# facebookresearch/NeRF-Det

Hardware: AMD Instinct MI355X
Metric: scenes/sec (50-view 240x320, 40x40x16 voxels) (higher is better)
Workload: dtype f32 (convolutions: fp32 operands as hi + lo fp16 pairs of the power-of-two pre-scaled tensors, three products per multiply on the fp16 MFMA, fp32 accumulate; error against fp64 at or below the six-product bf16x3 form's; a device-side range guard repeats a scene on bf16x3 when part of a tensor falls ; 1 GPU; cfg2: nerfdet_res50_2x_low_res forward_test, 50 views 240x320, 40x40x16 voxels, fp32, 1 scene/step/GPU, random-init weights; parallelism=scene replicas x1 (no data-path collective)

## Files before the change

include/nerfdet_hip.h:

```cpp
#ifndef NERFDET_HIP_H
#define NERFDET_HIP_H

#include <stdint.h>

#ifdef __cplusplus
extern "C" {
#endif

#define NDET_OK 0
#define NDET_E_INVALID (-1)
#define NDET_E_UNSUPPORTED (-2)
#define NDET_E_LAUNCH (-3)

#define NDET_LAYOUT_CN 0
#define NDET_LAYOUT_NC 1

int ndet_version(void);
const char* ndet_last_error(void);

int ndet_get_points(float* points, int nx, int ny, int nz, const float* voxel_size_host,
                    const float* origin_host, void* stream);

int ndet_nchw_to_nhwc(const float* src, float* dst, int n, int c, int hw, void* stream);

int ndet_hbm_copy(const float* src, float* dst, int64_t n_floats, void* stream);

int ndet_backproject(const float* features, int n_views, int C, int h, int w,
                     int64_t sv, int64_t sc, int64_t sy, int64_t sx,
                     const float* points, int N, const float* projection,
                     float* volume, uint8_t* valid, void* stream);

int ndet_backproject_aggregate(const float* features_nhwc, int n_views, int C, int h, int w,
                               int64_t view_pitch, int64_t row_pitch,
                               const float* points, int N, const float* projection,
                               const float* alpha, float* out, int out_layout, int64_t* count,
                               void* stream);

int ndet_density_features(const float* mapped_nhwc, int n_views, int cm, int h, int w,
                          int64_t mview_pitch, int64_t mrow_pitch, const float* bias,
                          const float* rgb, int H, int W, int64_t rsv, int64_t rsc, int64_t rsy,
                          const float* points, int N, const float* projection, const float* rgb_projection,
                          float* global_feat, void* stream);

int ndet_density_features_packed(const float* mapped_nhwc, int n_views, int cm, int h, int w,
                                 int64_t mview_pitch, int64_t mrow_pitch, const float* bias,
                                 const float* rgb, int H, int W, int64_t rsv, int64_t rsc, int64_t rsy,
                                 const float* points, int N, const float* projection,
                                 const float* rgb_projection, float* global_feat, void* stream);

typedef struct NdetDepthGate {
    int32_t size;
    int32_t dtype;
    int32_t n_views;
    int32_t h, w;
    int32_t H, W;
    const void* depth_f;
    int64_t f_view_pitch, f_row_pitch;
    const void* depth_r;
    int64_t r_view_pitch, r_row_pitch;
    double band;
} NdetDepthGate;

int ndet_depth_resize(const void* depth, int dtype, int n_views, int Hd, int Wd, int64_t sv, int64_t sy,
                      void* out_f, int h, int w, void* out_r, int H, int W, void* stream);

int ndet_backproject_gated(const float* features, int n_views, int C, int h, int w,
                           int64_t sv, int64_t sc, int64_t sy, int64_t sx,
                           const float* points, int N, const float* projection,
                           float* volume, uint8_t* valid, const NdetDepthGate* gate, void* stream);

int ndet_backproject_aggregate_gated(const float* features_nhwc, int n_views, int C, int h, int w,
                                     int64_t view_pitch, int64_t row_pitch,
                                     const float* points, int N, const float* projection,
                                     const float* alpha, float* out, int out_layout, int64_t* count,
                                     const NdetDepthGate* gate, void* stream);

int ndet_density_features_gated(const float* mapped_nhwc, int n_views, int cm, int h, int w,
                                int64_t mview_pitch, int64_t mrow_pitch, const float* bias,
                                const float* rgb, int H, int W, int64_t rsv, int64_t rsc, int64_t rsy,
                                const float* points, int N, const float* projection, const float* rgb_projection,
                                float* global_feat, const NdetDepthGate* gate, void* stream);

int ndet_density_features_packed_gated(const float* mapped_nhwc, int n_views, int cm, int h, int w,
                                       int64_t mview_pitch, int64_t mrow_pitch, const float* bias,
                                       const float* rgb, int H, int W, int64_t rsv, int64_t rsc, int64_t rsy,
                                       const float* points, int N, const float* projection,
                                       const float* rgb_projection, float* global_feat, const NdetDepthGate* gate, void* stream);

typedef struct NdetSceneAccum {
    int32_t size;
    int32_t N, C, cm;
    int32_t n_views;
    float* k1_sum;
    int64_t k1_pitch;
    int32_t* k1_count;
    float* k2_sum;
    int64_t k2_pitch;
    int32_t* k2_count;
} NdetSceneAccum;

int ndet_scene_accumulate(const NdetSceneAccum* s, const float* features_nhwc, int n_views, int h, int w,
                          int64_t view_pitch, int64_t row_pitch, const float* mapped_nhwc, int64_t mview_pitch,
                          int64_t mrow_pitch, const float* bias, const float* rgb, int H, int W, int64_t rsv, int64_t rsc,
                          int64_t rsy, const float* points, const float* projection, const float* rgb_projection,
                          const NdetDepthGate* gate, void* stream);

int ndet_scene_density_finish(const NdetSceneAccum* s, const float* bias, float* global_feat, void* stream);

int ndet_scene_volume_finish(const NdetSceneAccum* s, const float* alpha, float* out, int64_t* count, void* stream);

#define NDET_RING_MAX 64

int ndet_scene_density_finish_ring(const NdetSceneAccum* segs, int n_segs, const float* bias, float* global_feat, void* stream);

int ndet_scene_volume_finish_ring(const NdetSceneAccum* segs, int n_segs, const float* alpha, float* out, int64_t* count, void* stream);

#define NDET_GROUP_MAX 64
typedef struct NdetSceneSlot {
    float* k1_sum;
    int32_t* k1_count;
    float* k2_sum;
    int32_t* k2_count;
    const float* points;
    int64_t reserved[3];
} NdetSceneSlot;

typedef struct NdetSceneGroup {
    int32_t size;
// ... 127 lines not shown

int ndet_sample_pdf(const float* bins, const float* weights, int R, int M, const float* u, int u_row_stride, int n_out, float* samples,
                    void* stream);

int ndet_importance_merge(const float* z_vals, const float* weights, const float* ray_o, const float* ray_d, int R, int S, const float* u,
                          int u_row_stride, int n_imp, float* z_out, float* pts_out, float* z_samples_out, void* stream);

int64_t ndet_conv3d_workspace_bytes(int D, int H, int W, int Cin, int Cout, int ksize, int stride, int splits);
int ndet_conv3d_ndhwc(const float* in, const float* w_packed, float* out, int D, int H, int W, int Cin, int Cout,
                      int ksize, int stride, int transposed, const float* scale, const float* shift,
                      const float* residual, int relu, int splits, int tile, void* workspace, void* stream);

int ndet_conv_ndhwc(const float* in, const float* w_packed, float* out, int D, int H, int W, int Cin, int Cout,
                    const int* kernel_host, const int* stride_host, const int* pad_host, const float* scale,
                    const float* shift, const float* residual, int residual_up2, int relu, int splits, int tile,
                    void* workspace, void* stream);

int ndet_split_weights_bf16x3(const float* w_packed, int taps, int Cout, int Cin, uint16_t* planes, void* stream);

int ndet_split_weights_bf16x3_torch(const float* w_torch, int taps, int Cout, int Cin, int adjoint, uint16_t* planes, void* stream);

int ndet_point_mlp_alpha(const float* points, const float* global_feat, int N, int F, int K0, int hidden, const uint16_t* const* w_planes_host,
                         const float* w_inv_scale_host, const float* const* bias_host, const float* w_sigma, const float* b_sigma,
                         float* raw_sigma, float* alpha, float* h_out, void* stream);

int ndet_split_weights_f16x2(const float* w_packed, int taps, int Cout, int Cin, float scale, uint16_t* planes, void* stream);

int ndet_amax_f32(const float* x, int64_t n, float* slot, void* stream);

int ndet_amax_slot_floats(void);

int ndet_measurement_knob(const char* name_host, int64_t value);

typedef struct NdetConvArgs {
    int32_t size;
    const float* in;
    const uint16_t* w_planes;
    float* out;
    int D, H, W, Cin, Cout;
    int kernel[3], stride[3], pad[3];
    int transposed;
    const float* scale;
    const float* shift;
    const float* residual;
    int residual_up2, relu, splits, tile, arith;
    const float* in_amax;
    float w_inv_scale;
    const float* w_amax;
    float* out_amax;
    void* workspace;
    unsigned* guard;
    float guard_l1, guard_tol;
    int keep_partials;
    const float* map_w;
    const float* map_b;
    float* map_out;
} NdetConvArgs;
int ndet_conv_split(const NdetConvArgs* a, void* stream);

int ndet_conv_split_batch(const NdetConvArgs* a, int batch, void* stream);

int ndet_conv_halo_patch(int tile, int D, int H, int W, const int* kernel, int* patch, int* looped);

#define NDET_TILE_DIRECT 1
#define NDET_TILE_OWNS_ROWS 2
#define NDET_TILE_ORDER2 4
int ndet_conv_tile_info(int tile, int* rows, int* cols, int* flags);

int ndet_conv_chain(const float* in, const uint16_t* w_planes, int D, int H, int W, int Cin, int Cmid, const int* kernel,
                    const int* stride, const int* pad, const float* scale1, const float* shift1, const uint16_t* w3_planes,
                    int Cout, const float* scale3, const float* shift3, const float* residual, int relu3, float* out,
                    int arith, const float* in_amax, float w1_inv_scale, float w3_inv_scale, float* out_amax, float guard_l1,
                    float guard_l1_3, float guard_tol, unsigned* guard, void* stream);

int ndet_bottleneck_f16x2(const float* x, int N, int H, int W, int Cin, int Cout, const uint16_t* w1_planes, float w1_inv_scale, const float* scale1,
                          const float* shift1, const uint16_t* w2_planes, float w2_inv_scale, const float* scale2, const float* shift2,
                          const uint16_t* w3_planes, float w3_inv_scale, const float* scale3, const float* shift3, const uint16_t* wd_planes,
                          float wd_inv_scale, const float* scale_d, const float* shift_d, const float* in_amax, float* out_amax, float* out,
                          const float* guard_l1_host, float guard_tol, unsigned* guard, void* stream);

int ndet_bn_relu_maxpool_nhwc(const float* x, const float* scale, const float* shift, int N, int H, int W, int C,
                              float* out, void* stream);

int ndet_stem_pack_weights(const float* w_64x3x7x7, uint16_t* planes , void* stream);
int ndet_stem_pack_weights_f16x2(const float* w_64x3x7x7, float scale, uint16_t* planes , void* stream);

int ndet_stem_conv_bn_relu_maxpool(const float* images, int N, int H, int W, int64_t stride_n, int64_t stride_c, int64_t stride_y,
                                   int64_t stride_x, const uint16_t* w_planes, float w_inv_scale, const float* scale, const float* shift, float* out, float* out_amax,
                                   void* stream);

int ndet_normalize_views(const uint8_t* frames_bgr, const int* ids, int n_sel, int H, int W, const double* mean_rgb,
                         const double* std_rgb, float* img, float* denorm, void* stream);

int ndet_target_rays(const uint8_t* frames_bgr, const int* target_ids, int n_targets, int H, int W, int margin,
                     const float* intrinsic_rows, const float* camrotc2w, const float* cam_lightpos, const double* mean_rgb,
                     const double* std_rgb, float* raydirs, float* lightpos, float* gt_images, void* stream);

int ndet_resize_normalize_views(const uint8_t* frames_bgr, const int* ids, int n_sel, int Hs, int Ws, int Hr, int Wr, int H, int W,
                                const double* mean_rgb, const double* std_rgb, float* img, float* denorm, uint8_t* resized_bgr,
                                void* stream);

int ndet_depth_frames(const uint16_t* frames_mm, const int* ids, int n_sel, int Hd, int Wd, int h, int w, int margin, double* out,
                      void* stream);

int ndet_positive_indices(const double* x, int64_t n, int64_t* indices, int64_t* count, void* workspace, void* stream);

// ... 83 lines not shown
```

nerf-det_amd/_lib.py:

```python
from __future__ import annotations

import ctypes
import os
from ctypes import c_char_p, c_float, c_int, c_int64, c_void_p

_HERE = os.path.dirname(os.path.abspath(__file__))
LIB_PATH = os.path.join(_HERE, "lib", "libnerfdet_hip.so")

NDET_LAYOUT_CN = 0
NDET_LAYOUT_NC = 1

_P = c_void_p
_F3 = ctypes.POINTER(c_float)


class NdetConvArgs(ctypes.Structure):
    _fields_ = ([("size", ctypes.c_int32), ("in_", _P), ("w_planes", _P), ("out", _P)] + [(f, c_int) for f in ("D", "H", "W", "Cin", "Cout")]
                + [(f, c_int * 3) for f in ("kernel", "stride", "pad")] + [("transposed", c_int), ("scale", _P), ("shift", _P), ("residual", _P)]
                + [(f, c_int) for f in ("residual_up2", "relu", "splits", "tile", "arith")] + [("in_amax", _P), ("w_inv_scale", c_float)]
                + [(f, _P) for f in ("w_amax", "out_amax", "workspace", "guard")] + [("guard_l1", c_float), ("guard_tol", c_float), ("keep_partials", c_int)]
                + [(f, _P) for f in ("map_w", "map_b", "map_out")])


class NdetDepthGate(ctypes.Structure):
    _fields_ = [(f, ctypes.c_int32) for f in ("size", "dtype", "n_views", "h", "w", "H", "W")] + [
        ("depth_f", _P), ("f_view_pitch", c_int64), ("f_row_pitch", c_int64),
        ("depth_r", _P), ("r_view_pitch", c_int64), ("r_row_pitch", c_int64), ("band", ctypes.c_double)]


class NdetSceneAccum(ctypes.Structure):
    _fields_ = [(f, ctypes.c_int32) for f in ("size", "N", "C", "cm", "n_views")] + [
        ("k1_sum", _P), ("k1_pitch", c_int64), ("k1_count", _P), ("k2_sum", _P), ("k2_pitch", c_int64), ("k2_count", _P)]


class NdetBankView(ctypes.Structure):
    _fields_ = [("feat", _P), ("rgb4", _P), ("ke", c_float * 12)]


NDET_GROUP_MAX = 64


class NdetSceneSlot(ctypes.Structure):
    _fields_ = [(f, _P) for f in ("k1_sum", "k1_count", "k2_sum", "k2_count", "points")] + [("reserved", c_int64 * 3)]


class NdetSceneGroup(ctypes.Structure):
    _fields_ = [(f, ctypes.c_int32) for f in ("size", "n_slots", "N", "C", "cm", "reserved")] + [
        ("k1_pitch", c_int64), ("k2_pitch", c_int64), ("table", _P)]


class NdetGroupSel(ctypes.Structure):
    _fields_ = [("size", ctypes.c_int32), ("n", ctypes.c_int32), ("slot", ctypes.c_int32 * NDET_GROUP_MAX),
                ("n_views", ctypes.c_int32 * NDET_GROUP_MAX)]


NDET_RING_MAX = 64
NDET_GROUP_POOL_MAX = NDET_GROUP_MAX * (NDET_RING_MAX + 1)


class NdetGroupRingSel(ctypes.Structure):
    _fields_ = [("size", ctypes.c_int32), ("n", ctypes.c_int32), ("n_segs", ctypes.c_int32 * NDET_GROUP_MAX),
                ("n_views", ctypes.c_int32 * NDET_GROUP_MAX)]


class NdetBankGroupSel(ctypes.Structure):
    _fields_ = [("size", ctypes.c_int32), ("n", ctypes.c_int32), ("views", _P * NDET_GROUP_MAX), ("n_views", ctypes.c_int32 * NDET_GROUP_MAX),
                ("n_points", ctypes.c_int32 * NDET_GROUP_MAX)]


_G = ctypes.POINTER(NdetDepthGate)
_GR = ctypes.POINTER(NdetGroupRingSel)
_S = ctypes.POINTER(NdetSceneAccum)
_SG = ctypes.POINTER(NdetSceneGroup)
_GS = ctypes.POINTER(NdetGroupSel)

SIGNATURES = {
    "ndet_version": ([], c_int),
    "ndet_last_error": ([], c_char_p),
    "ndet_get_points": ([_P, c_int, c_int, c_int, _F3, _F3, _P], c_int),
    "ndet_nchw_to_nhwc": ([_P, _P, c_int, c_int, c_int, _P], c_int),
    "ndet_hbm_copy": ([_P, _P, c_int64, _P], c_int),
    "ndet_backproject": ([_P, c_int, c_int, c_int, c_int, c_int64, c_int64, c_int64, c_int64, _P, c_int, _P, _P, _P, _P], c_int),
    "ndet_backproject_aggregate": ([_P, c_int, c_int, c_int, c_int, c_int64, c_int64, _P, c_int, _P, _P, _P, c_int, _P, _P], c_int),
    "ndet_density_features": ([_P, c_int, c_int, c_int, c_int, c_int64, c_int64, _P, _P, c_int, c_int, c_int64, c_int64,
                               c_int64, _P, c_int, _P, _P, _P, _P], c_int),
    "ndet_density_features_packed": ([_P, c_int, c_int, c_int, c_int, c_int64, c_int64, _P, _P, c_int, c_int, c_int64, c_int64,
                                      c_int64, _P, c_int, _P, _P, _P, _P], c_int),
    "ndet_depth_resize": ([_P, c_int, c_int, c_int, c_int, c_int64, c_int64, _P, c_int, c_int, _P, c_int, c_int, _P], c_int),
    "ndet_backproject_gated": ([_P, c_int, c_int, c_int, c_int, c_int64, c_int64, c_int64, c_int64, _P, c_int, _P, _P, _P, _G, _P], c_int),
    "ndet_backproject_aggregate_gated": ([_P, c_int, c_int, c_int, c_int, c_int64, c_int64, _P, c_int, _P, _P, _P, c_int, _P, _G, _P], c_int),
    "ndet_density_features_gated": ([_P, c_int, c_int, c_int, c_int, c_int64, c_int64, _P, _P, c_int, c_int, c_int64, c_int64,
                                     c_int64, _P, c_int, _P, _P, _P, _G, _P], c_int),
    "ndet_density_features_packed_gated": ([_P, c_int, c_int, c_int, c_int, c_int64, c_int64, _P, _P, c_int, c_int, c_int64, c_int64,
                                            c_int64, _P, c_int, _P, _P, _P, _G, _P], c_int),
    "ndet_backproject_aggregate_bwd_gated": ([_P, c_int, c_int, c_int, c_int, c_int, c_int64, c_int64, _P, c_int, _P, _P, _G, _P], c_int),
    "ndet_density_features_bwd_gated": ([_P, _P, c_int, c_int, c_int, c_int, c_int64, c_int64, _P, _P, c_int, _P, _P, _P, _G, _P], c_int),
    "ndet_scene_accumulate": ([_S, _P, c_int, c_int, c_int, c_int64, c_int64, _P, c_int64, c_int64, _P, _P, c_int, c_int, c_int64, c_int64, c_int64,
                               _P, _P, _P, _G, _P], c_int),
    "ndet_scene_density_finish": ([_S, _P, _P, _P], c_int),
    "ndet_scene_volume_finish": ([_S, _P, _P, _P, _P], c_int),
    "ndet_scene_density_finish_ring": ([_S, c_int, _P, _P, _P], c_int),
    "ndet_scene_volume_finish_ring": ([_S, c_int, _P, _P, _P, _P], c_int),
    "ndet_scene_group_check": ([_SG, _GS, c_int], c_int),
    "ndet_scene_accumulate_group": ([_SG, _GS, c_int, _P, c_int, c_int, c_int64, c_int64, _P, c_int64, c_int64, _P, _P, c_int, c_int, c_int64, c_int64,
                                     c_int64, _P, _P, _G, _P], c_int),
    "ndet_scene_density_finish_group": ([_SG, _GS, _P, _P, _P], c_int),
    "ndet_scene_volume_finish_group": ([_SG, _GS, _P, _P, _P, _P], c_int),
    "ndet_scene_group_ring_check": ([_SG, _GR, _P], c_int),
    "ndet_scene_density_finish_group_ring": ([_SG, _GR, _P, _P, _P, _P, _P], c_int),
    "ndet_scene_volume_finish_group_ring": ([_SG, _GR, _P, _P, _P, _P, _P, _P], c_int),
    "ndet_alpha_gate": ([_P, _P, _P, _P, c_int, c_int, c_int, _P], c_int),
    "ndet_sigma_to_alpha": ([_P, _P, c_int, _P], c_int),
    "ndet_posenc_concat": ([_P, _P, c_int, c_int, c_int, _P, _P], c_int),
    "ndet_sigma_head": ([_P, c_int, _P, c_int, c_int, _P, _P, c_int, _P, _P, _P], c_int),
    "ndet_nms_workspace_bytes": ([c_int], c_int64),
    "ndet_aligned_3d_nms": ([_P, _P, _P, c_int, c_float, _P, _P, _P, _P], c_int),
    "ndet_head_decode": ([_P, c_int, _P, _P, c_int, c_int, c_int, _F3, _F3, _P, _P, _P, _P], c_int),
    "ndet_head_decode_levels": ([c_int, _P, _P, _P, _P, _P, _P, c_int, _P, c_int, c_int, c_int, _P, _P, _P, _P], c_int),
    "ndet_sample_along_rays": ([_P, _P, c_int, c_int, c_float, c_float, _P, _P, _P, _P], c_int),
    "ndet_ray_view_stats": ([_P, c_int, _P, c_int, c_float, c_float, _P, c_int, c_int, c_int64, c_int64, c_int64,
                             _P, c_int, c_int, c_int, c_int64, c_int64, _P, _P, _P, _P], c_int),
    "ndet_pack_rgb_nhwc4": ([_P, c_int, c_int, c_int, c_int64, c_int64, c_int64, _P, _P], c_int),
    "ndet_ray_view_stats_packed": ([_P, c_int, _P, c_int, c_float, c_float, _P, c_int, c_int, _P, c_int, c_int, c_int, c_int64, c_int64,
                                    _P, _P, _P, _P], c_int),
    "ndet_ray_view_stats_bank": ([_P, c_int, _P, c_int, c_float, c_float, c_int, c_int, c_int, c_int, c_int, _P, _P, _P, _P], c_int),
    "ndet_ray_view_stats_bank_group": ([_P, ctypes.POINTER(NdetBankGroupSel), c_float, c_float, c_int, c_int, c_int, c_int, c_int, _P, _P, _P, _P], c_int),
    "ndet_ray_view_stats_packed_bwd": ([_P, _P, c_int, _P, c_int, c_float, c_float, _P, c_int, c_int, c_int, c_int64, c_int64, _P, _P], c_int),
    "ndet_project_sample": ([_P, c_int, _P, c_int, c_float, c_float, _P, c_int, c_int, c_int64, c_int64, c_int64,
                             _P, c_int, c_int, c_int, c_int64, c_int64, _P, _P, _P], c_int),
    "ndet_composite": ([_P, _P, _P, c_int, c_int, c_int, _P, _P, _P, _P, _P, _P, _P, _P], c_int),
    "ndet_sample_pdf": ([_P, _P, c_int, c_int, _P, c_int, c_int, _P, _P], c_int),
    "ndet_importance_merge": ([_P, _P, _P, _P, c_int, c_int, _P, c_int, c_int, _P, _P, _P, _P], c_int),
    "ndet_backproject_aggregate_bwd": ([_P, c_int, c_int, c_int, c_int, c_int, c_int64, c_int64, _P, c_int, _P, _P, _P], c_int),
    "ndet_density_features_bwd": ([_P, _P, c_int, c_int, c_int, c_int, c_int64, c_int64, _P, _P, c_int, _P, _P, _P, _P], c_int),
    "ndet_ray_view_stats_bwd": ([_P, _P, c_int, _P, c_int, c_float, c_float, _P, c_int, c_int, c_int, c_int64, c_int64, _P, _P], c_int),
    "ndet_composite_bwd": ([_P, _P, _P, c_int, c_int, c_int, _P, _P, _P, _P, _P], c_int),
    "ndet_split_weights_bf16x3": ([_P, c_int, c_int, c_int, _P, _P], c_int),
    "ndet_split_weights_f16x2": ([_P, c_int, c_int, c_int, c_float, _P, _P], c_int),
    "ndet_conv_split": ([ctypes.POINTER(NdetConvArgs), _P], c_int),
    "ndet_conv_split_batch": ([ctypes.POINTER(NdetConvArgs), c_int, _P], c_int),
    "ndet_conv_halo_patch": ([c_int] * 4 + [ctypes.POINTER(c_int)] * 3, c_int),
    "ndet_conv_tile_info": ([c_int] + [ctypes.POINTER(c_int)] * 3, c_int),
    "ndet_conv_chain": ([_P, _P] + [c_int] * 5 + [_P] * 6 + [c_int, _P, _P, _P, c_int, _P, c_int, _P, c_float, c_float, _P, c_float, c_float, c_float, _P, _P], c_int),
# ... 105 lines not shown
```

nerf-det_amd/conv3d.py:

```python
from __future__ import annotations

import ctypes
import math
import struct
from ctypes import c_void_p
from dataclasses import dataclass
from typing import Optional, Sequence

import torch
from torch import nn

from . import _lib, conv_tiles, trace
from ._lib import _ptr, check, i3, raw_stream
from .conv_tuning import TUNED, TUNED_BF16, TUNED_F16, TUNED_SPLIT

ARITHMETIC = "f16x2"
F16_MIN_KSTEPS = 4
SPLIT_FAMILY = ("bf16x3", "bf16", "f16x2")
ARITH_ID = {"bf16x3": 0, "f16x2": 1, "bf16": 2}


def set_arithmetic(mode: str) -> str:
    global ARITHMETIC
    if mode not in ("f32", "bf16x3", "bf16", "f16x2"):
# ... 123 lines not shown

def amax_value(slot: torch.Tensor) -> float:
    return float(slot.view(-1, 32)[:, 0].max())


def tilemin_value(slot: torch.Tensor) -> float:
    v = int(slot.view(torch.int32).view(-1, 32)[:, 1].max())
    return 0.0 if v == 0 else struct.unpack("<f", struct.pack("<I", 0x7f800000 - v))[0]


_slot_width_checked = False


def amax_of(x: torch.Tensor) -> torch.Tensor:
    global amax_fallbacks, _slot_width_checked
    if not _slot_width_checked:
        assert _lib.load().ndet_amax_slot_floats() == _AmaxSlots.WIDTH, "amax slot width of the library differs from conv3d._AmaxSlots.WIDTH"
        _slot_width_checked = True
    slot = _amax_tag(x)
    if slot is None:
        amax_fallbacks += 1
        slot = AMAX.take(x.device)
        st = c_void_p(raw_stream(x.device))
        check(_lib.load().ndet_amax_f32(_ptr(x), x.numel(), _ptr(slot), st), "amax_f32")
        _tag_amax(x, slot, produced=False)
    return slot


GUARD_ENABLED = True
GUARD_TOL = 2.0 ** -15
guard_trips = 0
_GUARD_WORDS = {}


def guard_word(device) -> Optional[torch.Tensor]:
    if not GUARD_ENABLED:
        return None
    key = (device, raw_stream(device))
    w = _GUARD_WORDS.get(key)
    if w is None:
        w = _GUARD_WORDS[key] = torch.zeros(1, dtype=torch.int32, device=device)
    return w


def guard_begin(device) -> None:
    w = guard_word(device)
    if w is not None:
        w.zero_()


def guard_tripped(device) -> bool:
    w = guard_word(device)
    return bool(w is not None and int(w.item()) & 1)


def guard_l1(pk: ConvPack) -> float:
    hit = pk.guard_l1
    if hit is None:
        w = pk.w.abs()
        wmax = w.max()
        tiny = ((w > 0) & (w < wmax * 2.0 ** -16)).sum(dim=(0, 2)).float()
        l1 = w.sum(dim=(0, 2)) + wmax * tiny
        if pk.scale is not None:
            l1 = l1 * pk.scale.abs()
        v = float(l1.max())
        hit = pk.guard_l1 = v if math.isfinite(v) else float("inf")
    return hit


launch_hook = None

KERNEL_NAMES = {("f32", 64): "k_conv3d_igemm<64,64,2,2>", ("f32", 128): "k_conv3d_igemm<128,128,4,2>"}
for _t, _row in conv_tiles.TILES.items():
    KERNEL_NAMES.update({("bf16x3", _t): _row.name, ("bf16", _t): _row.name, ("f16x2", _t): _row.name + "/f16x2"})


def _launch(flops, thunk, arith="f32", tile=0, nbytes=0, name=None):
    name = name or KERNEL_NAMES.get((arith, tile), f"{arith}:{tile}")
    if launch_hook is not None:
        return launch_hook(flops, thunk, name)
    return trace.span(name, thunk, flops=flops, bytes=nbytes, kind="conv")


def choose_tiling(m: int, cout: int, k_iters: int, tile: int = 0, splits: int = 0, transposed: bool = False):
    if tile == 0 and splits == 0:
        hit = TUNED.get((m, cout, k_iters, int(transposed)))
        if hit is not None:
            return hit
    if tile == 0:
        big = ((m + 127) // 128) * ((cout + 127) // 128)
        tile = 128 if (big >= 120 and cout >= 128 and k_iters > 4) else 64
    if splits == 0:
        if transposed:
            return tile, 1
        tiles = ((m + tile - 1) // tile) * ((cout + tile - 1) // tile)
        cap = 1200 if tile == 128 else 2400
        splits = 1
        while splits < 8 and k_iters // (splits + 1) >= 64 and tiles * (splits + 1) <= cap:
            splits += 1
    return tile, splits


def choose_tiling_split(m: int, cout: int, k_iters: int, tile: int = 0, splits: int = 0, transposed: bool = False, halo_ok: bool = False):
    if tile == 0 and splits in (0, 1):
        key = (m, cout, k_iters, int(transposed))
        hit = (TUNED_BF16.get(key) if ARITHMETIC == "bf16" else TUNED_F16.get(key) if ARITHMETIC == "f16x2" else None) or TUNED_SPLIT.get(key)
# ... 42 lines not shown


def f16_weight_scale(wmax: float) -> float:
    if not (wmax > 0.0 and math.isfinite(wmax)):
        return 1.0
    e = max(math.frexp(wmax)[1], -96)
    return math.ldexp(1.0, 15 - e)


def split_planes_f16(pk: ConvPack):
    hit = pk.planes_f16
    if hit is None:
        w = pk.w
        taps, cout, cin = w.shape
        if cin % 32:
            raise ValueError(f"conv_ndhwc_arith: Cin={cin} must be a multiple of 32")
        scale = f16_weight_scale(float(w.abs().max()))
        planes = torch.empty((taps, cin // 32, 2, cout, 32), dtype=torch.int16, device=w.device)
        st = c_void_p(raw_stream(w.device))
        check(_lib.load().ndet_split_weights_f16x2(_ptr(w), taps, cout, cin, scale, _ptr(planes), st), "split_weights_f16x2")
        hit = pk.planes_f16 = (planes, 1.0 / scale)
    return hit


def layer_arithmetic(k_iters: int) -> str:
    if ARITHMETIC == "f16x2" and k_iters < F16_MIN_KSTEPS:
        return "bf16x3"
    return ARITHMETIC


def _conv_split(x, pk, out, dims, kernel, stride, pad, transposed, residual, residual_up2, relu, splits, tile, m, k_iters, flops, want_amax=True, chain=None,
                keep_partials=False, batch=1):
    assert batch == 1 or (chain is None and not keep_partials and not residual_up2 and pk.w_amax is None)
    halo_ok = (not transposed and all(s == 1 for s in stride) and all(k % 2 == 1 and q == k // 2 for k, q in zip(kernel, pad))
               and kernel[0] * kernel[1] * kernel[2] > 1)
    tile, splits = choose_tiling_split(m, pk.cout, k_iters, tile, 1 if (transposed or residual_up2) else splits, transposed, halo_ok)
    tile, splits = conv_tiles.resolve(tile, splits, m=m, cout=pk.cout, cin=pk.cin, taps=kernel[0] * kernel[1] * kernel[2], transposed=transposed,
                                      halo_ok=halo_ok, direct_epilogue=DIRECT_EPILOGUE, batch=batch)
    ws = torch.empty((m * pk.cout * splits * 4,), dtype=torch.uint8, device=x.device) if splits > 1 else None
    st = c_void_p(raw_stream(x.device))
    lib = _lib.load()
    d, h, w = dims
    nbytes = 4 * (x.numel() + pk.w.numel() + out.numel() + (0 if residual is None else residual.numel()))
    arith = layer_arithmetic(k_iters)
    if ARITHMETIC == "f16x2" and pk.arith:
        arith = pk.arith
        want_amax = want_amax and pk.keep_amax
    if NO_AMAX_COMMIT:
        want_amax = False
    a = _lib.NdetConvArgs(size=ctypes.sizeof(_lib.NdetConvArgs), in_=x.data_ptr(), out=out.data_ptr(), D=d, H=h, W=w, Cin=pk.cin, Cout=pk.cout,
                          kernel=kernel, stride=stride, pad=pad, transposed=int(transposed), scale=_addr(pk.scale), shift=_addr(pk.shift),
                          residual=_addr(residual), residual_up2=int(residual_up2), relu=relu, splits=splits, tile=tile, arith=ARITH_ID[arith],
                          workspace=_addr(ws))
    keep, mapped = False, None
    if ARITHMETIC != "f16x2":
        a.w_planes = split_planes(pk).data_ptr()
        want_amax = False
    elif arith == "f16x2" and pk.w_amax is not None:
        assert not transposed and not residual_up2
        keep = keep_partials
        want_amax = want_amax and not keep
        a.w_planes, a.in_amax, a.w_amax, a.keep_partials = pk.planes_f16[0].data_ptr(), amax_of(x).data_ptr(), pk.w_amax.data_ptr(), int(keep)
        gw = guard_word(x.device) if pk.guard else None
        a.guard, a.guard_l1, a.guard_tol = _addr(gw), float(kernel[0] * kernel[1] * kernel[2] * pk.cin), GUARD_TOL
    else:
        if arith == "f16x2":
            planes, a.w_inv_scale = split_planes_f16(pk)
            a.in_amax = amax_of(x).data_ptr()
            gw = guard_word(x.device)
        else:
            planes, gw = split_planes(pk), None
        a.w_planes, a.guard, a.guard_l1, a.guard_tol = planes.data_ptr(), _addr(gw), (guard_l1(pk) if gw is not None else 0.0), GUARD_TOL
        if (chain is not None and conv_tiles.owns_rows(tile) and splits == 1 and residual is None and relu == 0 and not transposed and pk.cout == 256
                and arith in ("f16x2", "bf16x3")):
            mapped = torch.empty((m, 32), dtype=torch.float32, device=x.device)
            a.map_w, a.map_b, a.map_out = chain[0].data_ptr(), chain[1].data_ptr(), mapped.data_ptr()
            nbytes += 4 * mapped.numel()
    out_amax = AMAX.take(x.device) if want_amax else None
    a.out_amax = _addr(out_amax)
    if batch == 1:
        _launch(flops, lambda: check(lib.ndet_conv_split(a, st), "conv_split"), arith, tile, nbytes)
    else:
        _launch(flops, lambda: check(lib.ndet_conv_split_batch(a, batch, st), "conv_split_batch"), arith, tile, nbytes,
                name=KERNEL_NAMES.get((arith, tile), f"{arith}:{tile}") + "/batch")
    if want_amax:
        _tag_amax(out, out_amax)
    if keep_partials:
        return out, ((ws.view(torch.float32), splits) if keep and splits > 1 else None)
    return out if mapped is None else (out, mapped)


def projection_ok() -> bool:
    return ARITHMETIC == "f16x2"


def _addr(t):
    return None if t is None else t.data_ptr()


def pack_weight(w: torch.Tensor, transposed: bool = False) -> torch.Tensor:
    if w.dim() == 4:
        cout, cin = w.shape[:2]
        return w.permute(2, 3, 0, 1).reshape(-1, cout, cin).contiguous().float()
    if transposed:
        cin, cout = w.shape[:2]
        return w.permute(2, 3, 4, 1, 0).reshape(-1, cout, cin).contiguous().float()
# ... 317 lines not shown
```

nerf-det_amd/csrc/conv_common.hpp:

```cpp
#pragma once
#include <type_traits>
#include "ndet_common.hpp"

#define CBK 32

struct Conv3dParams {
    const float* in;
    const float* w;
    float* out;
    const float* scale;
    const float* shift;
    const float* res;
    float* partial;
    int D, H, W, Cin;
    int OD, OH, OW, Cout;
    int kd, kh, kw;
    int sd, sh, sw;
    int pd, ph, pw;
    int relu;
    int transposed;
    int splits;
    int M;
    int res_up2;
    int RH, RW;
    int max_order;
    int direct = 0;
    int order = 0;
    const float* amax_in = nullptr;
    float winv = 1.0f;
    const float* w_amax = nullptr;
    int nt = 0;
    float* amax_out = nullptr;
    const float* map_w = nullptr;
    const float* map_b = nullptr;
    float* map_out = nullptr;
    unsigned* guard = nullptr;
    float guard_l1 = 0.0f;
    float guard_tol = 0.0f;
};


#define NDET_AMAX_SUB 8
#define NDET_AMAX_STRIDE 32
__device__ __forceinline__ unsigned conv_xcc_id() { return __builtin_amdgcn_s_getreg((3 << 11) | 20) & 7u; }

__device__ __forceinline__ float conv_amax_read(const float* slot) {
    float v = slot[(threadIdx.x & (NDET_AMAX_SUB - 1)) * NDET_AMAX_STRIDE];
#pragma unroll
    for (int o = NDET_AMAX_SUB / 2; o; o >>= 1) v = fmaxf(v, __shfl_xor(v, o));
    return __uint_as_float(__builtin_amdgcn_readfirstlane(__float_as_uint(v)));
}

__device__ __forceinline__ float conv_xscale_of(float amax) {
    int eb = (int)((__float_as_uint(amax) >> 23) & 0xffu);
    eb = eb < 30 ? 30 : eb;
    return __uint_as_float((unsigned)(268 - eb) << 23);
}
__device__ __forceinline__ float conv_xinv_of(float amax) {
    int eb = (int)((__float_as_uint(amax) >> 23) & 0xffu);
    eb = eb < 30 ? 30 : eb;
    return __uint_as_float((unsigned)(eb - 14) << 23);
}
__device__ __forceinline__ float conv_xscale(const float* amax) { return conv_xscale_of(conv_amax_read(amax)); }
__device__ __forceinline__ float conv_winv(const Conv3dParams& p) { return p.w_amax ? conv_xinv_of(conv_amax_read(p.w_amax)) : p.winv; }
__device__ __forceinline__ float conv_oscale(const Conv3dParams& p) { return p.amax_in ? conv_xinv_of(conv_amax_read(p.amax_in)) * conv_winv(p) : 1.0f; }
__device__ __forceinline__ float conv_amax_in(const Conv3dParams& p) { return p.amax_in ? conv_amax_read(p.amax_in) : 0.0f; }
__device__ __forceinline__ float conv_oscale_of(const Conv3dParams& p, float amax_in) { return p.amax_in ? conv_xinv_of(amax_in) * conv_winv(p) : 1.0f; }

__device__ __forceinline__ void conv_amax_commit(float* slot, float mx) {
    __shared__ float wg_amax[16];
#pragma unroll
    for (int o = 32; o; o >>= 1) mx = fmaxf(mx, __shfl_xor(mx, o));
    const int nw = ((int)blockDim.x + 63) >> 6;
    if ((threadIdx.x & 63) == 0) wg_amax[threadIdx.x >> 6] = mx;
    __syncthreads();
    if (threadIdx.x == 0) {
        for (int i = 1; i < nw; ++i) mx = fmaxf(mx, wg_amax[i]);
        const unsigned bits = __float_as_uint(mx);
        unsigned* sub = reinterpret_cast<unsigned*>(slot) + conv_xcc_id() * NDET_AMAX_STRIDE;
        if (bits) atomicMax(sub, bits);
        if (bits && bits <= 0x7f800000u) atomicMax(sub + 1, 0x7f800000u - bits);
    }
}

__device__ __forceinline__ void conv_amax_commit_tiles(float* slot, float mx, float tmin) {
    __shared__ float wg_tmax[16], wg_tmin[16];
#pragma unroll
    for (int o = 32; o; o >>= 1) { mx = fmaxf(mx, __shfl_xor(mx, o)); tmin = fminf(tmin, __shfl_xor(tmin, o)); }
    const int nw = ((int)blockDim.x + 63) >> 6;
    if ((threadIdx.x & 63) == 0) { wg_tmax[threadIdx.x >> 6] = mx; wg_tmin[threadIdx.x >> 6] = tmin; }
    __syncthreads();
// ... 125 lines not shown
                                                int ztap, int zsplit, float& mx, float osc) {
    conv_store_rows_mapped<BN, NTHR>(p, Cs, cld, rows, n0, tid, ztap, zsplit, ConvLinearRows{m_first}, mx, osc);
}
template <int BN, int NTHR, typename RowMap>
__device__ __forceinline__ void conv_map_rows(const Conv3dParams& p, float* Cs, int cld, int tid, RowMap m_of, float osc, const float* Wl) {
    constexpr int KS = NTHR >= 1024 ? 8 : 4;
    static_assert(BN % KS == 0 && NTHR >= 128 * KS, "conv_map_rows: 128 threads per channel slice");
    constexpr int KQ = BN / KS;
    float acc[4][4];
#pragma unroll
    for (int i = 0; i < 4; ++i)
#pragma unroll
        for (int j = 0; j < 4; ++j) acc[i][j] = 0.f;
    const int kq = tid >> 7, rg = (tid >> 3) & 15, jg = tid & 7;
    if (tid < 128 * KS) {
        const float* c = Cs + rg * cld + kq * KQ;
        const float* w = Wl + (kq * KQ) * 32 + 4 * jg;
#pragma unroll 2
        for (int k = 0; k < KQ; ++k) {
            const float4 wv = *reinterpret_cast<const float4*>(w + k * 32);
#pragma unroll
            for (int i = 0; i < 4; ++i) {
                const float v = c[(16 * i) * cld + k];
                acc[i][0] = fmaf(v, wv.x, acc[i][0]); acc[i][1] = fmaf(v, wv.y, acc[i][1]);
                acc[i][2] = fmaf(v, wv.z, acc[i][2]); acc[i][3] = fmaf(v, wv.w, acc[i][3]);
            }
        }
    }
    __syncthreads();
    float* P = Cs;
    if (tid < 128 * KS) {
#pragma unroll
        for (int i = 0; i < 4; ++i)
            *reinterpret_cast<float4*>(P + ((kq * 64 + rg + 16 * i) * 32 + 4 * jg)) = make_float4(acc[i][0], acc[i][1], acc[i][2], acc[i][3]);
    }
    __syncthreads();
    for (int o = tid; o < 64 * 8; o += NTHR) {
        const int row = o >> 3, j4 = o & 7;
        const int m = m_of(row);
        if (m < 0 || m >= p.M) continue;
        float4 t = *reinterpret_cast<const float4*>(P + (row * 32 + 4 * j4));
#pragma unroll
        for (int q = 1; q < KS; ++q) {
            const float4 u = *reinterpret_cast<const float4*>(P + ((q * 64 + row) * 32 + 4 * j4));
            t.x += u.x; t.y += u.y; t.z += u.z; t.w += u.w;
        }
        const float4 b = *reinterpret_cast<const float4*>(p.map_b + 4 * j4);
        *reinterpret_cast<float4*>(p.map_out + (int64_t)m * 32 + 4 * j4) = make_float4(fmaf(t.x, osc, b.x), fmaf(t.y, osc, b.y), fmaf(t.z, osc, b.z), fmaf(t.w, osc, b.w));
    }
    __syncthreads();
}

__device__ __forceinline__ bool conv_writes_final(const Conv3dParams& p) { return p.transposed || p.splits <= 1; }
```

nerf-det_amd/csrc/conv_split_kernels.hip:

```cpp
#include "conv_common.hpp"

#include "spl_common.hpp"

#include <type_traits>

template <int BM, int BN, int WGM, int WGN, int SCH, bool BATCH = false>
__device__ __forceinline__ void conv_split_mainloop(const Conv3dParams& p, const uint16_t* __restrict__ wsplit, uint16_t* lds16,
                                                    f32x16 (&acc)[BM / WGM / 32][BN / WGN / 32], int& ztap) {
    constexpr int NTHR = 64 * WGM * WGN;
    constexpr int WM = BM / WGM, WN = BN / WGN;
    constexpr int MT = WM / 32, NT = WN / 32;
    constexpr int RPA = NTHR / 8;
    constexpr int RPB = NTHR / 4;
    constexpr int AR = BM / RPA, BR = BN / RPB;
    static_assert(AR >= 1 && BR >= 1 && MT >= 1 && NT >= 1, "tile too small for the thread count");
    constexpr int APL = BM * SPL_RS, BPL = BN * SPL_RS;
    constexpr int NPL = Spl<SCH>::NPL, WPL = Spl<SCH>::WPL;
    const float xs = SCH == 1 ? conv_xscale(p.amax_in) : 1.0f;
    uint16_t* As = lds16;
    uint16_t* Bs = lds16 + NPL * APL;

    const int tid = threadIdx.x;
    const int lane = tid & 63, wave = tid >> 6;
    const int wm = wave / WGN, wn = wave % WGN;
// ... 110 lines not shown
            uint16_t* dst = Bs + (brow_ + RPB * i) * SPL_RS + bkg * 8;
#pragma unroll
            for (int pl = 0; pl < NPL; ++pl) *reinterpret_cast<uint4*>(dst + pl * BPL) = rb[i][pl];
        }
    };

    if (it_begin < it_end) {
        load_tile();
        store_tile();
    }
    __syncthreads();

    const int frow = lane & 31, fk = (lane >> 5) * 8;
    const uint16_t* abase = As + (wm * WM + frow) * SPL_RS + fk;
    const uint16_t* bbase = Bs + (wn * WN + frow) * SPL_RS + fk;
    for (int it = it_begin; it < it_end; ++it) {
        const bool more = it + 1 < it_end;
        if (more) load_tile();
#pragma unroll
        for (int ks = 0; ks < CBK / 16; ++ks) {
            bf16x8 fa[NPL][MT], fb[NPL][NT];
#pragma unroll
            for (int pl = 0; pl < NPL; ++pl) {
                const int pq = NPL - 1 - pl;
#pragma unroll
                for (int t = 0; t < MT; ++t) fa[pl][t] = *reinterpret_cast<const bf16x8*>(abase + pl * APL + t * 32 * SPL_RS + ks * 16);
#pragma unroll
                for (int t = 0; t < NT; ++t) fb[pq][t] = *reinterpret_cast<const bf16x8*>(bbase + pq * BPL + t * 32 * SPL_RS + ks * 16);
            }
#pragma unroll
            for (int order = NPL - 1; order >= 0; --order)
                if (order <= p.max_order)
#pragma unroll
                for (int pa = 0; pa <= order; ++pa) {
                    const int pb = order - pa;
#pragma unroll
                    for (int ta = 0; ta < MT; ++ta)
#pragma unroll
                        for (int tb = 0; tb < NT; ++tb)
                            acc[ta][tb] = spl_mfma32<SCH>(fa[pa][ta], fb[pb][tb], acc[ta][tb]);
                }
        }
        __syncthreads();
        if (more) store_tile();
        __syncthreads();
    }
}

#ifndef UNI128_F16_WGS
#define UNI128_F16_WGS 3
#endif
template <int BM, int BN, int SCH> constexpr int uni_min_wgs() { return (SCH == 1 && BM == 128 && BN == 128) ? UNI128_F16_WGS : 2; }
#define SPL_BATCH 4
template <int BM, int BN, int WGM, int WGN, int SCHB = 0>
__global__ __launch_bounds__(64 * WGM * WGN, (uni_min_wgs<BM, BN, (SCHB & 3)>())) void k_conv_split(const Conv3dParams p, const uint16_t* __restrict__ wsplit) {
    constexpr int SCH = SCHB & 3;
    constexpr bool BATCH = (SCHB & SPL_BATCH) != 0;
    constexpr int NTHR = 64 * WGM * WGN;
    constexpr int WM = BM / WGM, WN = BN / WGN, MT = WM / 32, NT = WN / 32;
    extern __shared__ __attribute__((aligned(16))) uint16_t lds16[];
    const int tid = threadIdx.x;
    const int lane = tid & 63, wave = tid >> 6;
    const int wm = wave / WGN, wn = wave % WGN;
    const ConvBlock blk = conv_block(p);
    const int m0 = blk.x * BM, n0 = blk.y * BN;
    f32x16 acc[MT][NT];
    int ztap;
    const float amax_in = conv_amax_in(p);
    conv_guard_check(p, amax_in);
    conv_split_mainloop<BM, BN, WGM, WGN, SCH, BATCH>(p, wsplit, lds16, acc, ztap);
    const float osc = conv_oscale_of(p, amax_in);

    if (p.direct) {
        float mx = 0.0f;
        const unsigned obytes = (unsigned)((int64_t)p.M * p.Cout * 4);
        const unsigned rbytes = p.res_up2 ? (unsigned)((int64_t)p.OD * p.RH * p.RW * p.Cout * 4) : obytes;
        const __amdgpu_buffer_rsrc_t rres = __builtin_amdgcn_make_buffer_rsrc((void*)(p.res ? p.res : p.out), 0, p.res ? rbytes : obytes, 0x00020000);
        const __amdgpu_buffer_rsrc_t rout = __builtin_amdgcn_make_buffer_rsrc((void*)p.out, 0, obytes, 0x00020000);
#pragma unroll
        for (int tb = 0; tb < NT; ++tb) {
            const int co = n0 + wn * WN + tb * 32 + (lane & 31);
            if (n0 + wn * WN + tb * 32 >= p.Cout) continue;
            const float sc = p.scale ? p.scale[co] : 1.0f, sh = p.scale ? p.shift[co] : 0.0f;
#pragma unroll
            for (int ta = 0; ta < MT; ++ta) {
                const int mrow = m0 + wm * WM + ta * 32 + 4 * (lane >> 5);
                const unsigned vo = (unsigned)(((int64_t)mrow * p.Cout + co) * 4);
                float rr[16];
                if (p.res && p.res_up2) {
                    int uw = mrow % p.OW, uh = (mrow / p.OW) % p.OH, ud = mrow / (p.OW * p.OH);
#pragma unroll
                    for (int r = 0; r < 16; ++r) {
                        if (r) {
                            uw += (r & 3) ? 1 : 5;
                            if (p.OW >= 5) { if (uw >= p.OW) { uw -= p.OW; if (++uh == p.OH) { uh = 0; ++ud; } } }
                            else while (uw >= p.OW) { uw -= p.OW; if (++uh == p.OH) { uh = 0; ++ud; } }
                        }
                        const unsigned ro = ((((unsigned)ud * p.RH + (uh >> 1)) * p.RW + (uw >> 1)) * p.Cout + co) * 4u;
                        rr[r] = __uint_as_float(__builtin_amdgcn_raw_buffer_load_b32(rres, (mrow + (r & 3) + 8 * (r >> 2) < p.M) ? ro : 0xfffffff0u, 0, 0));
                    }
                } else {
#pragma unroll
                    for (int r = 0; r < 16; ++r) {
                        const unsigned so = __builtin_amdgcn_readfirstlane((unsigned)(((r & 3) + 8 * (r >> 2)) * p.Cout * 4));
                        rr[r] = p.res ? __uint_as_float(__builtin_amdgcn_raw_buffer_load_b32(rres, vo, so, 0)) : 0.0f;
                    }
                }
#pragma unroll
                for (int r = 0; r < 16; ++r) {
                    const unsigned so = __builtin_amdgcn_readfirstlane((unsigned)(((r & 3) + 8 * (r >> 2)) * p.Cout * 4));
                    float v = (acc[ta][tb][r] * osc) * sc + sh;
                    if (p.relu == 2) v = fmaxf(v, 0.f);
                    v += rr[r];
                    if (p.relu == 1) v = fmaxf(v, 0.f);
                    if (p.nt) __builtin_amdgcn_raw_buffer_store_b32(__float_as_uint(v), rout, vo, so, 2);
                    else __builtin_amdgcn_raw_buffer_store_b32(__float_as_uint(v), rout, vo, so, 0);
                    if (mrow + (r & 3) + 8 * (r >> 2) < p.M) mx = fmaxf(mx, fabsf(v));
                }
            }
        }
        if (p.amax_out) conv_amax_commit(p.amax_out, mx);
        return;
    }
    constexpr int CLDC = BN + 4;
    float* Cs = reinterpret_cast<float*>(lds16);
    float mx = 0.0f;
    for (int h = 0; h < WGM; ++h) {
        if (wm == h) {
#pragma unroll
            for (int ta = 0; ta < MT; ++ta)
#pragma unroll
                for (int tb = 0; tb < NT; ++tb)
#pragma unroll
                    for (int r = 0; r < 16; ++r)
                        Cs[(ta * 32 + (r & 3) + 8 * (r >> 2) + 4 * (lane >> 5)) * CLDC + wn * WN + tb * 32 + (lane & 31)] = acc[ta][tb][r];
        }
        __syncthreads();
        conv_store_rows<BN, NTHR>(p, Cs, CLDC, m0 + h * WM, WM, n0, tid, ztap, blk.z, mx, osc);
        __syncthreads();
    }
    if (p.amax_out && conv_writes_final(p)) conv_amax_commit(p.amax_out, mx);
}


struct ConvChain {
    const uint16_t* w3;
    float w3inv;
    float* amax_out;
    const float* scale3;
    const float* shift3;
    const float* res;
    float* out;
    int Cout3;
    int relu3;
    float guard_l1 = 0.0f;
};

#ifndef CHAIN64_F16_WGS
#define CHAIN64_F16_WGS 4
#endif
template <int MID, int SCH>
__global__ __launch_bounds__(256, MID == 64 ? (SCH == 1 ? CHAIN64_F16_WGS : 3) : 2) void k_conv_split_chain(const Conv3dParams p, const uint16_t* __restrict__ wsplit, const ConvChain c) {
    constexpr int BM = 128, BN = MID, WGM = 2, WGN = 2;
    constexpr int WM = BM / WGM, WN = BN / WGN, MT = WM / 32, NT = WN / 32;
    constexpr int NPL = Spl<SCH>::NPL, WPL = Spl<SCH>::WPL;
    constexpr int YRS = MID;
    constexpr int HALVES = MID == 128 ? 2 : 1;
    constexpr int RH = BM / HALVES;
    constexpr int YPL = RH * YRS;
    constexpr int NRT = RH / 32;
    constexpr int KS = MID / 16;
    constexpr int KG = 4, NKG = KS / KG;
    extern __shared__ __attribute__((aligned(16))) uint16_t lds16[];
    const int tid = threadIdx.x;
    const int lane = tid & 63, wave = __builtin_amdgcn_readfirstlane(tid >> 6);
    const int wm = wave / WGN, wn = wave % WGN;
    const int m0 = blockIdx.x * BM;
    f32x16 acc[MT][NT];
    int ztap;
    const float amax_in = conv_amax_in(p);
    conv_guard_check(p, amax_in);
    conv_split_mainloop<BM, BN, WGM, WGN, SCH>(p, wsplit, lds16, acc, ztap);
    const float osc = conv_oscale_of(p, amax_in);

    float ys = 1.0f, osc3 = 1.0f;
    if constexpr (SCH == 1) {
        const float osc1 = conv_oscale(p);
        float ymax = 0.0f;
#pragma unroll
        for (int ta = 0; ta < MT; ++ta)
#pragma unroll
            for (int tb = 0; tb < NT; ++tb) {
// ... 290 lines not shown
                    fa[pl][t] = *reinterpret_cast<const bf16x8*>(abase + pl * APL + t * 32 * SPL_RS + (((2 * ks + (lane >> 5)) ^ (((wm * WM + t * 32 + frow) >> 4) & 3)) << 3));
#pragma unroll
                for (int t = 0; t < NT; ++t) fb[pl][t] = *reinterpret_cast<const bf16x8*>(bbase + pl * BPL + t * 32 * SPL_RS + ks * 16);
            }
#pragma unroll
            for (int order = NPL - 1; order >= 0; --order)
                if (order <= p.max_order)
#pragma unroll
                for (int pa = 0; pa <= order; ++pa) {
                    const int pb = order - pa;
#pragma unroll
                    for (int ta_ = 0; ta_ < MT; ++ta_)
#pragma unroll
                        for (int tb_ = 0; tb_ < NT; ++tb_)
                            acc[ta_][tb_] = spl_mfma32<SCH>(fa[pa][ta_], fb[pb][tb_], acc[ta_][tb_]);
                }
        }
        __syncthreads();
        if (more) store_tile();
        __syncthreads();
    }
    constexpr int CLDC = BN + 4;
    float* Cs = reinterpret_cast<float*>(lds16);
    for (int h = 0; h < WGM; ++h) {
        if (wm == h) {
#pragma unroll
            for (int ta_ = 0; ta_ < MT; ++ta_)
#pragma unroll
                for (int tb_ = 0; tb_ < NT; ++tb_)
#pragma unroll
                    for (int r = 0; r < 16; ++r)
                        Cs[(ta_ * 32 + (r & 3) + 8 * (r >> 2) + 4 * (lane >> 5)) * CLDC + wn * WN + tb_ * 32 + (lane & 31)] = acc[ta_][tb_][r];
        }
        __syncthreads();
        float mx_unused = 0.0f;
        conv_store_rows<BN, NTHR>(p, Cs, CLDC, m0 + h * WM, WM, n0, tid, 0, bz, mx_unused, osc);
        __syncthreads();
    }
}


typedef unsigned int u32x4 __attribute__((ext_vector_type(4)));
typedef float f32x4v __attribute__((ext_vector_type(4)));
__device__ __forceinline__ int ws_swz(int row) { return (row >> 1) & 2; }
__device__ __forceinline__ void spl_dma16(__amdgpu_buffer_rsrc_t rsrc, uint16_t* lds_dst, unsigned voffset, unsigned soffset) {
    __builtin_amdgcn_raw_ptr_buffer_load_lds(rsrc, (__attribute__((address_space(3))) void*)lds_dst, 16, voffset, soffset, 0, 0);
}

#define WS_BM 128
#define WS_BN 256
#define WS_DEPTH 2
#define WS_OOB 0x80000000u

template <int SCHB>
__global__ __launch_bounds__(512, 1) void k_conv_split_ws(const Conv3dParams p, const uint16_t* __restrict__ wsplit) {
    constexpr int SCH = SCHB & 3;
    constexpr bool BATCH = (SCHB & SPL_BATCH) != 0;
    constexpr int APL = WS_BM * CBK, BPL = WS_BN * CBK;
    constexpr int NPL = Spl<SCH>::NPL, WPL = Spl<SCH>::WPL;
    constexpr int STAGE = NPL * (APL + BPL);
    constexpr int AR = 4, BR = 4;
    extern __shared__ __attribute__((aligned(16))) uint16_t lds16[];

    const int tid = threadIdx.x;
    const int lane = tid & 63;
    const int wave = __builtin_amdgcn_readfirstlane(tid >> 6);
    const bool consumer = wave < 4;
    const int wm = (wave & 3) >> 1, wn = wave & 1;
    const ConvBlock blk = conv_block(p);
    const int m0 = blk.x * WS_BM, n0 = blk.y * WS_BN;
    const float amax_in = conv_amax_in(p);
    conv_guard_check(p, amax_in);
    const int stid = tid & 255;
    const int akq = stid & 7, arow_ = stid >> 3;
    const int bkg = stid & 3, brow_ = stid >> 2;

    const int cin_steps = p.Cin / CBK;
    const int wkd = p.transposed ? 1 : p.kd, wkh = p.transposed ? 1 : p.kh, wkw = p.transposed ? 1 : p.kw;
    const int taps = wkd * wkh * wkw;
    const int n_iters_all = taps * cin_steps;
    int it_begin = 0, it_end = n_iters_all;
    int ztap = 0;
    if (p.transposed) {
        ztap = blk.z;
    } else if (p.splits > 1) {
        const int s = blk.z;
        it_begin = (int)((int64_t)n_iters_all * s / p.splits);
        it_end = (int)((int64_t)n_iters_all * (s + 1) / p.splits);
    }
    const int n_it = it_end - it_begin;
    const int n_round = (n_it + WS_DEPTH - 1) / WS_DEPTH * WS_DEPTH;

    f32x4v acc[4][8];
#pragma unroll
    for (int a = 0; a < 4; ++a)
#pragma unroll
        for (int b = 0; b < 8; ++b) acc[a][b] = (f32x4v){0.f, 0.f, 0.f, 0.f};

    if (!consumer) {
        const int64_t shift = p.transposed ? 0 : (((int64_t)p.pd * p.H + p.ph) * p.W + p.pw) * p.Cin;
        const __amdgpu_buffer_rsrc_t ares = __builtin_amdgcn_make_buffer_rsrc((void*)(p.in - shift), 0, WS_OOB, 0x00020000);
        const __amdgpu_buffer_rsrc_t bres = __builtin_amdgcn_make_buffer_rsrc((void*)wsplit, 0, WS_OOB, 0x00020000);
        unsigned avoff[AR], amask[AR];
#pragma unroll
        for (int i = 0; i < AR; ++i) {
            const int m = m0 + arow_ + 32 * i;
            const bool vok = m < p.M;
// ... 117 lines not shown
        }
    } else {
        const int frow = lane & 15, fc = lane >> 4;
        const int kc = (fc ^ ws_swz(frow)) * 8;
        const int aoff = (wm * 64 + frow) * CBK + kc;
        const int boff = NPL * APL + (wn * 128 + frow) * CBK + kc;
        __syncthreads();
        for (int j = 0; j < n_round; ++j) {
            if (j < n_it) {
                const uint16_t* st = lds16 + (j & 1) * STAGE;
                bf16x8 fa[NPL][4], fb[NPL][8];
#pragma unroll
                for (int pl = 0; pl < NPL; ++pl) {
                    const int pq = NPL - 1 - pl;
#pragma unroll
                    for (int t = 0; t < 4; ++t) fa[pl][t] = *reinterpret_cast<const bf16x8*>(st + aoff + pl * APL + t * 16 * CBK);
#pragma unroll
                    for (int t = 0; t < 8; ++t) fb[pq][t] = *reinterpret_cast<const bf16x8*>(st + boff + pq * BPL + t * 16 * CBK);
                }
#pragma unroll
                for (int order = NPL - 1; order >= 0; --order)
                    if (order <= p.max_order)
#pragma unroll
                    for (int pa = 0; pa <= order; ++pa) {
                        const int pb = order - pa;
#pragma unroll
                        for (int ta = 0; ta < 4; ++ta)
#pragma unroll
                            for (int tb = 0; tb < 8; ++tb)
                                acc[ta][tb] = spl_mfma16<SCH>(fa[pa][ta], fb[pb][tb], acc[ta][tb]);
                    }
            }
            __syncthreads();
        }
    }

    constexpr int CLDC = WS_BN + 4;
    float* Cs = reinterpret_cast<float*>(lds16);
    float mx = 0.0f;
    for (int h = 0; h < 2; ++h) {
        if (consumer && wm == h) {
#pragma unroll
            for (int ta = 0; ta < 4; ++ta)
#pragma unroll
                for (int tb = 0; tb < 8; ++tb)
#pragma unroll
                    for (int r = 0; r < 4; ++r)
                        Cs[(ta * 16 + (lane >> 4) * 4 + r) * CLDC + wn * 128 + tb * 16 + (lane & 15)] = acc[ta][tb][r];
        }
        __syncthreads();
        conv_store_rows<WS_BN, 512>(p, Cs, CLDC, m0 + h * 64, 64, n0, tid, ztap, blk.z, mx, conv_oscale_of(p, amax_in));
        __syncthreads();
    }
    if (p.amax_out && conv_writes_final(p)) conv_amax_commit(p.amax_out, mx);
}

static inline int conv_scheme(const Conv3dParams& p) { return p.max_order == 0 ? 2 : (p.max_order == 1 ? 1 : 0); }

template <class F>
static inline int with_scheme(int sch, F&& f) {
    return sch == 2 ? f(std::integral_constant<int, 2>{}) : (sch == 1 ? f(std::integral_constant<int, 1>{}) : f(std::integral_constant<int, 0>{}));
}

template <bool BATCH>
static int split_launch_ws_n(const Conv3dParams& p, int batch, hipStream_t st, const char* fn) {
    const int taps = p.transposed ? 1 : p.kd * p.kh * p.kw;
    const int64_t nvol = BATCH ? batch : 1;
    NDET_REQUIRE(taps <= 32, NDET_E_UNSUPPORTED, "%s: the 128x256 tile supports at most 32 taps", fn);
    NDET_REQUIRE(nvol * p.D * p.H * p.W * p.Cin * 4 < ((int64_t)1 << 31) && (int64_t)(p.transposed ? 8 : taps) * p.Cin * p.Cout * 6 < ((int64_t)1 << 31),
                 NDET_E_UNSUPPORTED, "%s: the 128x256 tile addresses at most 2 GB per operand", fn);
    const int zdim = p.transposed ? 8 : p.splits;
    dim3 grid((p.M + WS_BM - 1) / WS_BM, (p.Cout + WS_BN - 1) / WS_BN, zdim);
    const int sch = conv_scheme(p);
    size_t lds = (size_t)2 * (sch == 2 ? 1 : (sch == 1 ? 2 : 3)) * (WS_BM + WS_BN) * CBK * sizeof(uint16_t);
    const size_t cs = (size_t)64 * (WS_BN + 4) * sizeof(float);
    if (cs > lds) lds = cs;
    return with_scheme(sch, [&](auto s) -> int {
        const auto kernel = k_conv_split_ws<decltype(s)::value + (BATCH ? SPL_BATCH : 0)>;
        NDET_RAISE_LDS(kernel, lds);
        hipLaunchKernelGGL(kernel, grid, dim3(512), lds, st, p, (const uint16_t*)p.w);
        return NDET_OK;
    });
}
static int split_launch_ws(const Conv3dParams& p, hipStream_t st, const char* fn) { return split_launch_ws_n<false>(p, 1, st, fn); }
static int split_launch_ws_batch(const Conv3dParams& p, int batch, hipStream_t st, const char* fn) { return split_launch_ws_n<true>(p, batch, st, fn); }


template <int OFF>
__device__ __forceinline__ void lds_store64_unseen(unsigned addr, uint2 v) {
    const unsigned long long d = ((unsigned long long)v.y << 32) | v.x;
    asm volatile("ds_write_b64 %0, %1 offset:%2" ::"v"(addr), "v"(d), "n"(OFF) : "memory");
}

#ifndef WSP_DEPTH
#define WSP_DEPTH 2
#endif
template <int SCH, int BM, int NCONS>
__global__ __launch_bounds__(64 * (NCONS + 4), 1) void k_conv_split_wsp(const Conv3dParams p, const uint16_t* __restrict__ wsplit, int n_mt, int n_nt) {
    static_assert((BM == 128 && (NCONS == 4 || NCONS == 8)) || (BM == 64 && NCONS == 4), "consumer layouts: 2 x 2 of 64 x 128, 2 x 4 of 64 x 64, 1 x 4 of 64 x 64");
    constexpr int CW = NCONS / (BM / 64);
    constexpr int WNC = WS_BN / CW, NTB = WNC / 16;
    constexpr int APL = BM * CBK, BPL = WS_BN * CBK;
    constexpr int NPL = Spl<SCH>::NPL, WPL = Spl<SCH>::WPL;
    constexpr int STAGE = NPL * (APL + BPL);
    extern __shared__ __attribute__((aligned(16))) uint16_t lds16[];

    const int tid = threadIdx.x;
    const int lane = tid & 63;
    const int wave = __builtin_amdgcn_readfirstlane(tid >> 6);
    const bool consumer = wave < NCONS;
    const float xs = SCH == 1 ? conv_xscale(p.amax_in) : 1.0f;
    const float osc = conv_oscale(p);
    if (SCH == 1) conv_guard_check(p, conv_amax_in(p));
    __shared__ float s_tmax[2][NCONS];
    const bool track = p.amax_out != nullptr && p.splits == 1;
    float mx = 0.0f, tmin = INFINITY;
    int kt = 0;
    auto fold_tile = [&](int k) {
        float m = s_tmax[k & 1][0];
#pragma unroll
        for (int i = 1; i < NCONS; ++i) m = fmaxf(m, s_tmax[k & 1][i]);
        if (m > 0.0f) tmin = fminf(tmin, m);
    };
    const int wm = (wave % NCONS) / CW, wn = (wave % NCONS) % CW;

    const int cin_steps = p.Cin / CBK;
    const int wkd = p.kd, wkh = p.kh, wkw = p.kw;
    const int taps = wkd * wkh * wkw;
    const int n_iters_all = taps * cin_steps;
    const int n_tiles = n_mt * n_nt * p.splits;
    const int G = gridDim.x;
// ... 241 lines not shown
    NDET_REQUIRE(taps <= 32, NDET_E_UNSUPPORTED, "%s: the persistent 128x256 tile supports at most 32 taps", fn);
    NDET_REQUIRE(p.Cout % 16 == 0, NDET_E_UNSUPPORTED, "%s: the persistent 128x256 tile needs Cout %% 16 == 0", fn);
    NDET_REQUIRE((int64_t)p.D * p.H * p.W * p.Cin * 4 < ((int64_t)1 << 31) && (int64_t)taps * p.Cin * p.Cout * 6 < ((int64_t)1 << 31) &&
                     ((int64_t)p.M + 128) * p.Cout * 4 < ((int64_t)1 << 31),
                 NDET_E_UNSUPPORTED, "%s: the persistent 128x256 tile addresses at most 2 GB per operand", fn);
    const int n_mt = (p.M + BM - 1) / BM, n_nt = (p.Cout + WS_BN - 1) / WS_BN;
    const int64_t n_tiles = (int64_t)n_mt * n_nt * p.splits;
    static int n_cu = 0;
    if (n_cu == 0) {
        int dev = 0;
        hipDeviceProp_t prop;
        if (hipGetDevice(&dev) != hipSuccess || hipGetDeviceProperties(&prop, dev) != hipSuccess) n_cu = 256;
        else n_cu = prop.multiProcessorCount > 0 ? prop.multiProcessorCount : 256;
    }
    const int grid = (int)(n_tiles < n_cu ? n_tiles : n_cu);
    const int sch = conv_scheme(p);
    const size_t lds = (size_t)2 * (sch == 2 ? 1 : (sch == 1 ? 2 : 3)) * (BM + WS_BN) * CBK * sizeof(uint16_t);
    return with_scheme(sch, [&](auto s) -> int {
        const auto kernel = k_conv_split_wsp<decltype(s)::value, BM, NCONS>;
        NDET_RAISE_LDS(kernel, lds);
        hipLaunchKernelGGL(kernel, dim3(grid), dim3(64 * (NCONS + 4)), lds, st, p, (const uint16_t*)p.w, n_mt, n_nt);
        return NDET_OK;
    });
}


struct HaloGeom {
    int ltd, lth, ltw;
    int npd, nph, npw;
    int HH, HW, NH;
    int T;
    int KDL;
    int Tin;
};

struct HaloRowMap {
    int first, ltw, lth, d0, h0, w0, OD, OH, OW;
    __device__ __forceinline__ int operator()(int row) const {
        const int r = first + row;
        const int tw = r & ((1 << ltw) - 1), th = (r >> ltw) & ((1 << lth) - 1), td = r >> (ltw + lth);
        const int od = d0 + td, oh = h0 + th, ow = w0 + tw;
        return (od < OD && oh < OH && ow < OW) ? (od * OH + oh) * OW + ow : -1;
    }
};
struct HaloRowMapBatch {
    HaloRowMap in_volume;
    int vol_first;
    __device__ __forceinline__ int operator()(int row) const {
        const int m = in_volume(row);
        return m < 0 ? m : vol_first + m;
    }
};

template <int NT16, int WGN, int SCHB, int NPROD = 4>
__global__ __launch_bounds__(64 * (2 * WGN + NPROD), 1) void k_conv_split_halo(const Conv3dParams p, const uint16_t* __restrict__ wsplit, const HaloGeom g) {
    constexpr int SCH = SCHB & 3;
    constexpr bool BATCH = (SCHB & SPL_BATCH) != 0;
    constexpr int BN = 16 * NT16 * WGN;
    constexpr int NCONS = 2 * WGN, NTHR = 64 * (NCONS + NPROD);
    constexpr int PT = 64 * NPROD;
    constexpr int HALO_MAX = (BN == 128) ? 400 : 224;
    constexpr int NSTAGE = (BN == 128) ? 3 : 2;
    constexpr int NPIECE = (HALO_MAX * 8 + PT - 1) / PT;
    constexpr int APL = HALO_MAX * CBK, BPL = BN * CBK;
    constexpr int NPL = SCH == 1 ? 2 : (SCH == 2 ? 1 : 3);
    constexpr int WPL = SCH == 1 ? 2 : 3;
    constexpr int BSTAGE = NPL * BPL;
    constexpr int BR = BN / (16 * NPROD);
    static_assert(BR >= 1 && BN % (16 * NPROD) == 0, "every producer wave stages 16 rows of each row group");
    constexpr int NB = NPL * BR;
    extern __shared__ __attribute__((aligned(16))) uint16_t lds16[];
    uint16_t* Bs = lds16 + NPL * APL;

    const int tid = threadIdx.x;
    const int lane = tid & 63;
    const int wave = __builtin_amdgcn_readfirstlane(tid >> 6);
    const bool consumer = wave < NCONS;
    const int wm = (wave % NCONS) / WGN, wn = (wave % NCONS) % WGN;
    const ConvBlock blk = conv_block(p);
    const int n0 = blk.y * BN;
    const int TH = 1 << g.lth, TW = 1 << g.ltw;
    int pb = blk.x;
    const int pwi = pb % g.npw; pb /= g.npw;
    const int phi = pb % g.nph;
    const int pdv = pb / g.nph;
    const int vol = BATCH ? pdv / g.npd : 0;
    const int pdi = BATCH ? pdv - vol * g.npd : pdv;
    const int d0 = pdi << g.ltd, h0 = phi << g.lth, w0 = pwi << g.ltw;
    const float amax_in = conv_amax_in(p);
    conv_guard_check(p, amax_in);

    const int nch_all = p.Cin / CBK;
    int cb = 0, ce = nch_all;
    if (p.splits > 1) {
        cb = (int)((int64_t)nch_all * blk.z / p.splits);
        ce = (int)((int64_t)nch_all * (blk.z + 1) / p.splits);
    }
    const int nch = ce - cb;
    const int T = g.T, Tin = g.Tin;
    const int S = nch * T;
    const int nphase = nch * g.KDL;

    f32x4v acc[4][NT16];
#pragma unroll
    for (int a = 0; a < 4; ++a)
#pragma unroll
        for (int b = 0; b < NT16; ++b) acc[a][b] = (f32x4v){0.f, 0.f, 0.f, 0.f};
// ... 127 lines not shown
                    const int pq = NPL - 1 - pl;
#pragma unroll
                    for (int ta = 0; ta < 4; ++ta) fa[pl][ta] = *reinterpret_cast<const bf16x8*>(ap[ta] + pl * APL);
#pragma unroll
                    for (int tb = 0; tb < NT16; ++tb) fb[pq][tb] = *reinterpret_cast<const bf16x8*>(bst + pq * BPL + tb * 16 * CBK);
                }
#pragma unroll
                for (int order = NPL - 1; order >= 0; --order)
                    if (order <= p.max_order)
#pragma unroll
                    for (int pa = 0; pa <= order; ++pa) {
                        const int pbb = order - pa;
#pragma unroll
                        for (int ta = 0; ta < 4; ++ta)
#pragma unroll
                            for (int tb = 0; tb < NT16; ++tb) {
                                acc[ta][tb] = spl_mfma16<SCH>(fa[pa][ta], fb[pbb][tb], acc[ta][tb]);
                            }
                    }
                if (++kw == wkw) {
                    kw = 0;
                    if (++kh == wkh) { kh = 0; ++kd; }
                }
                __syncthreads();
            }
            if (ci + 1 < nphase) __syncthreads();
        }
    }
    __builtin_amdgcn_s_setprio(0);

    constexpr int CLDC = BN + 4;
    float* Cs = reinterpret_cast<float*>(lds16);
    float mx = 0.0f;
    for (int h = 0; h < 2; ++h) {
        if (consumer && wm == h) {
#pragma unroll
            for (int ta = 0; ta < 4; ++ta)
#pragma unroll
                for (int tb = 0; tb < NT16; ++tb)
#pragma unroll
                    for (int r = 0; r < 4; ++r)
                        Cs[(ta * 16 + (lane >> 4) * 4 + r) * CLDC + wn * (16 * NT16) + tb * 16 + (lane & 15)] = acc[ta][tb][r];
        }
        __syncthreads();
        const HaloRowMap rmap{h * 64, g.ltw, g.lth, d0, h0, w0, p.OD, p.OH, p.OW};
        const float osc = conv_oscale_of(p, amax_in);
        float* Wl = Cs + 64 * CLDC;
        if (p.map_out && h == 0)
            for (int i = tid; i < BN * 8; i += NTHR) reinterpret_cast<float4*>(Wl)[i] = reinterpret_cast<const float4*>(p.map_w)[i];
        if constexpr (BATCH) conv_store_rows_mapped<BN, NTHR>(p, Cs, CLDC, 64, n0, tid, 0, blk.z, HaloRowMapBatch{rmap, vol * p.OD * p.OH * p.OW}, mx, osc);
        else conv_store_rows_mapped<BN, NTHR>(p, Cs, CLDC, 64, n0, tid, 0, blk.z, rmap, mx, osc);
        __syncthreads();
        if (p.map_out) conv_map_rows<BN, NTHR>(p, Cs, CLDC, tid, rmap, osc, Wl);
    }
    if (p.amax_out && conv_writes_final(p)) conv_amax_commit(p.amax_out, mx);
}

static bool halo_geometry(const Conv3dParams& p, int halo_max, HaloGeom& g) {
    double best = 1e30;
    for (int dloop = 0; dloop <= (p.kd > 1 ? 1 : 0); ++dloop)
        for (int ltd = 0; ltd <= 7; ++ltd)
            for (int lth = 0; lth + ltd <= 7; ++lth) {
                const int ltw = 7 - ltd - lth;
                const int TD = 1 << ltd, TH = 1 << lth, TW = 1 << ltw;
                const int HD = dloop ? TD : TD + p.kd - 1, HH = TH + p.kh - 1, HW = TW + p.kw - 1;
                const int NH = HD * HH * HW;
                if (NH > halo_max) continue;
                const int npd = (p.OD + TD - 1) / TD, nph = (p.OH + TH - 1) / TH, npw = (p.OW + TW - 1) / TW;
                const double waste = (double)npd * TD * nph * TH * npw * TW / ((double)p.OD * p.OH * p.OW);
                const int kdl = dloop ? p.kd : 1;
                const double cost = waste * (1.0 + 0.03 * NH * kdl / 128.0);
                if (cost < best) {
                    best = cost;
                    g.ltd = ltd; g.lth = lth; g.ltw = ltw; g.npd = npd; g.nph = nph; g.npw = npw; g.HH = HH; g.HW = HW; g.NH = NH;
                    g.KDL = kdl;
                }
            }
    g.T = p.kd * p.kh * p.kw;
    g.Tin = g.T / (best < 1e29 ? g.KDL : 1);
    return best < 1e29;
}

template <int NT16, int WGN, int SCH, int NPROD, bool BATCH>
static int split_launch_halo(const Conv3dParams& p, int batch, hipStream_t st, const char* fn) {
    constexpr int NPL = SCH == 1 ? 2 : (SCH == 2 ? 1 : 3);
    constexpr int BN = 16 * NT16 * WGN, HALO_MAX = (BN == 128) ? 400 : 224, NSTAGE = (BN == 128) ? 3 : 2;
    NDET_REQUIRE(!p.transposed && p.sd == 1 && p.sh == 1 && p.sw == 1 && (p.kd & 1) && (p.kh & 1) && (p.kw & 1) && p.pd == p.kd / 2 &&
                     p.ph == p.kh / 2 && p.pw == p.kw / 2,
                 NDET_E_UNSUPPORTED, "%s: the halo tile needs a stride-1 same-padded convolution with odd kernel extents", fn);
    const int64_t nvol = BATCH ? batch : 1;
    NDET_REQUIRE(nvol * p.D * p.H * p.W * p.Cin * 4 < ((int64_t)1 << 31) && (int64_t)p.kd * p.kh * p.kw * p.Cin * p.Cout * 6 < ((int64_t)1 << 31),
                 NDET_E_UNSUPPORTED, "%s: the halo tile addresses at most 2 GB per operand", fn);
    NDET_REQUIRE(p.splits <= p.Cin / CBK, NDET_E_INVALID, "%s: the halo tile splits K over the %d channel chunks only", fn, p.Cin / CBK);
    HaloGeom g;
    NDET_REQUIRE(halo_geometry(p, HALO_MAX, g), NDET_E_UNSUPPORTED, "%s: no patch shape fits the halo tile", fn);
    dim3 grid((unsigned)(nvol * g.npd * g.nph * g.npw), (p.Cout + BN - 1) / BN, p.splits);
    size_t lds = (size_t)(NPL * HALO_MAX * CBK + NSTAGE * NPL * BN * CBK) * sizeof(uint16_t);
    const size_t cs = (size_t)64 * (BN + 4) * sizeof(float);
    if (cs > lds) lds = cs;
    const size_t lds_map = cs + (size_t)BN * 32 * sizeof(float);
    const size_t lds_cap = lds_map > lds ? lds_map : lds;
    if (p.map_out) {
        NDET_REQUIRE(p.Cout == BN && p.splits == 1 && !p.res && p.relu == 0, NDET_E_UNSUPPORTED,
                     "%s: the chained projection needs a tile that owns all %d output channels of its rows, no split-K / residual / ReLU", fn, p.Cout);
        lds = lds_cap;
    }
    const auto kernel = k_conv_split_halo<NT16, WGN, SCH + (BATCH ? SPL_BATCH : 0), NPROD>;
    NDET_RAISE_LDS(kernel, lds_cap);
    hipLaunchKernelGGL(kernel, grid, dim3(64 * (2 * WGN + NPROD)), lds, st, p, (const uint16_t*)p.w, g);
    return NDET_OK;
}

template <int BM, int BN, int WGM, int WGN, int SCH, bool BATCH>
static int split_launch_tile_sch(const Conv3dParams& p, hipStream_t st, const char* fn) {
    const int zdim = p.transposed ? 8 : p.splits;
    dim3 grid((p.M + BM - 1) / BM, (p.Cout + BN - 1) / BN, zdim);
    size_t lds = (size_t)Spl<SCH>::NPL * (BM + BN) * SPL_RS * sizeof(uint16_t);
    const size_t cs = (size_t)(BM / WGM) * (BN + 4) * sizeof(float);
    if (cs > lds) lds = cs;
    const auto kernel = k_conv_split<BM, BN, WGM, WGN, SCH + (BATCH ? SPL_BATCH : 0)>;
    if (lds > 64 * 1024) NDET_RAISE_LDS(kernel, lds);
    hipLaunchKernelGGL(kernel, grid, dim3(64 * WGM * WGN), lds, st, p, (const uint16_t*)p.w);
    return NDET_OK;
}
template <int BM, int BN, int WGM, int WGN>
static int split_launch_tile(const Conv3dParams& p, hipStream_t st, const char* fn) {
    return with_scheme(conv_scheme(p), [&](auto s) { return split_launch_tile_sch<BM, BN, WGM, WGN, decltype(s)::value, false>(p, st, fn); });
}
template <int BM, int BN, int WGM, int WGN>
static int split_launch_tile_batch(const Conv3dParams& p, int, hipStream_t st, const char* fn) {
    return with_scheme(conv_scheme(p), [&](auto s) { return split_launch_tile_sch<BM, BN, WGM, WGN, decltype(s)::value, true>(p, st, fn); });
}
template <int NT16, int WGN>
static int split_launch_halo_any(const Conv3dParams& p, hipStream_t st, const char* fn) {
    return with_scheme(conv_scheme(p), [&](auto s) { return split_launch_halo<NT16, WGN, decltype(s)::value, 4, false>(p, 1, st, fn); });
}
template <int NT16, int WGN>
static int split_launch_halo_any_batch(const Conv3dParams& p, int batch, hipStream_t st, const char* fn) {
    return with_scheme(conv_scheme(p), [&](auto s) { return split_launch_halo<NT16, WGN, decltype(s)::value, 4, true>(p, batch, st, fn); });
}
static int split_launch_halo_p8(const Conv3dParams& p, hipStream_t st, const char* fn) {
    return with_scheme(conv_scheme(p), [&](auto s) {
        constexpr int SCH = decltype(s)::value;
        return split_launch_halo<4, 4, SCH, SCH == 0 ? 4 : 8, false>(p, 1, st, fn);
    });
}
static int split_launch_halo_p8_batch(const Conv3dParams& p, int batch, hipStream_t st, const char* fn) {
    return with_scheme(conv_scheme(p), [&](auto s) {
        constexpr int SCH = decltype(s)::value;
        return split_launch_halo<4, 4, SCH, SCH == 0 ? 4 : 8, true>(p, batch, st, fn);
    });
}

#ifndef NDET_ORDER_DEFAULT
#define NDET_ORDER_DEFAULT -1
#endif
static int64_t g_nt_bytes = (int64_t)32 << 20;
static bool g_order2 = true;
static int64_t conv_nt_bytes() { return g_nt_bytes; }
static int g_wgrad_wide = 1;
static int g_wgrad_xcd = 1;

extern "C" int ndet_measurement_knob(const char* name, int64_t value) {
    const char* fn = "ndet_measurement_knob";
    NDET_REQUIRE(name, NDET_E_INVALID, "%s: null name", fn);
    if (!strcmp(name, "nt_bytes")) { NDET_REQUIRE(value >= 0, NDET_E_INVALID, "%s: nt_bytes must be >= 0", fn); g_nt_bytes = value; return NDET_OK; }
    if (!strcmp(name, "order2")) { NDET_REQUIRE(value == 0 || value == 1, NDET_E_INVALID, "%s: order2 is 0 or 1", fn); g_order2 = value != 0; return NDET_OK; }
    if (!strcmp(name, "deterministic_scatter")) { NDET_REQUIRE(value == 0 || value == 1, NDET_E_INVALID, "%s: deterministic_scatter is 0 or 1", fn); g_ndet_deterministic_scatter = (int)value; return NDET_OK; }
    if (!strcmp(name, "wgrad_wide")) { NDET_REQUIRE(value == 0 || value == 1, NDET_E_INVALID, "%s: wgrad_wide is 0 or 1", fn); g_wgrad_wide = (int)value; return NDET_OK; }
    if (!strcmp(name, "wgrad_xcd")) { NDET_REQUIRE(value == 0 || value == 1, NDET_E_INVALID, "%s: wgrad_xcd is 0 or 1", fn); g_wgrad_xcd = (int)value; return NDET_OK; }
    ndet_set_error("%s: unknown knob '%s' (nt_bytes, order2, deterministic_scatter, wgrad_wide, wgrad_xcd)", fn, name);
    return NDET_E_INVALID;
}
extern "C" int ndet_amax_slot_floats(void) { return NDET_AMAX_SUB * NDET_AMAX_STRIDE; }

struct ConvTile {
    int id, rows, cols, flags;
    int (*launch)(const Conv3dParams&, hipStream_t, const char*);
    int (*launch_batch)(const Conv3dParams&, int batch, hipStream_t, const char*);
};
static const ConvTile CONV_TILES[] = {
    {64, 64, 64, NDET_TILE_ORDER2, split_launch_tile<64, 64, 2, 2>, split_launch_tile_batch<64, 64, 2, 2>},
    {128, 128, 128, NDET_TILE_ORDER2, split_launch_tile<128, 128, 2, 2>, split_launch_tile_batch<128, 128, 2, 2>},
    {12864, 128, 64, NDET_TILE_ORDER2, split_launch_tile<128, 64, 2, 2>, split_launch_tile_batch<128, 64, 2, 2>},
    {100064, 64, 64, NDET_TILE_ORDER2 | NDET_TILE_DIRECT, split_launch_tile<64, 64, 2, 2>, split_launch_tile_batch<64, 64, 2, 2>},
    {100128, 128, 128, NDET_TILE_ORDER2 | NDET_TILE_DIRECT, split_launch_tile<128, 128, 2, 2>, split_launch_tile_batch<128, 128, 2, 2>},
    {112864, 128, 64, NDET_TILE_ORDER2 | NDET_TILE_DIRECT, split_launch_tile<128, 64, 2, 2>, split_launch_tile_batch<128, 64, 2, 2>},
    {128256, 128, 256, NDET_TILE_ORDER2, split_launch_ws, split_launch_ws_batch},
    {129256, 128, 256, 0, split_launch_wsp<128, 4>, nullptr},
    {129257, 128, 256, 0, split_launch_wsp<128, 8>, nullptr},
    {129064, 64, 256, 0, split_launch_wsp<64, 4>, nullptr},
    {3128, 128, 128, 0, split_launch_halo_any<4, 2>, split_launch_halo_any_batch<4, 2>},
    {3256, 128, 256, NDET_TILE_OWNS_ROWS, split_launch_halo_any<8, 2>, split_launch_halo_any_batch<8, 2>},
    {3257, 128, 256, NDET_TILE_OWNS_ROWS, split_launch_halo_any<4, 4>, split_launch_halo_any_batch<4, 4>},
    {3258, 128, 256, NDET_TILE_OWNS_ROWS, split_launch_halo_p8, split_launch_halo_p8_batch},
};
static const ConvTile* conv_tile(int id) {
    for (const ConvTile& t : CONV_TILES)
        if (t.id == id) return &t;
    return nullptr;
}

extern "C" int ndet_conv_tile_info(int tile, int* rows, int* cols, int* flags) {
    const char* fn = "ndet_conv_tile_info";
    NDET_REQUIRE(rows && cols && flags, NDET_E_INVALID, "%s: null pointer", fn);
    const ConvTile* t = conv_tile(tile);
    NDET_REQUIRE(t, NDET_E_INVALID, "%s: unknown tile %d", fn, tile);
    *rows = t->rows; *cols = t->cols; *flags = t->flags;
    return NDET_OK;
}

extern "C" int ndet_conv_halo_patch(int tile, int D, int H, int W, const int* kernel, int* patch, int* looped) {
    const char* fn = "ndet_conv_halo_patch";
    NDET_REQUIRE(kernel && patch && looped, NDET_E_INVALID, "%s: null pointer", fn);
    const ConvTile* t = conv_tile(tile);
    NDET_REQUIRE(t && (tile == 3128 || (t->flags & NDET_TILE_OWNS_ROWS)), NDET_E_INVALID, "%s: tile %d is not a halo tile", fn, tile);
    NDET_REQUIRE(D > 0 && H > 0 && W > 0 && kernel[0] >= 1 && kernel[1] >= 1 && kernel[2] >= 1, NDET_E_INVALID, "%s: sizes must be positive", fn);
    Conv3dParams p{};
    p.OD = D; p.OH = H; p.OW = W; p.kd = kernel[0]; p.kh = kernel[1]; p.kw = kernel[2];
    HaloGeom g;
    NDET_REQUIRE(halo_geometry(p, t->cols == 128 ? 400 : 224, g), NDET_E_UNSUPPORTED, "%s: no patch shape fits the halo tile", fn);
    patch[0] = 1 << g.ltd; patch[1] = 1 << g.lth; patch[2] = 1 << g.ltw;
    *looped = g.KDL > 1 ? 1 : 0;
    return NDET_OK;
}

static int conv_split_launch_n(Conv3dParams& p, int tile, bool keep_partials, int batch, hipStream_t st, const char* fn) {
    p.nt = (p.splits <= 1 || p.transposed) && (int64_t)p.M * p.Cout * 4 * (p.transposed ? 8 : 1) >= conv_nt_bytes() ? 1 : 0;
    const int64_t big_tiles = (int64_t)((p.M + 127) / 128) * ((p.Cout + 127) / 128);
    if (tile == 0) tile = (big_tiles >= 192 && p.Cout >= 128) ? 128 : 64;
    const ConvTile* t = conv_tile(tile);
    NDET_REQUIRE(t, NDET_E_INVALID, "%s: unknown tile %d", fn, tile);
    NDET_REQUIRE(batch == 1 || t->launch_batch, NDET_E_UNSUPPORTED, "%s: tile %d takes one volume per launch", fn, tile);
    p.direct = (t->flags & NDET_TILE_DIRECT) ? 1 : 0;
    NDET_REQUIRE(!p.direct || (!p.transposed && p.splits == 1 && p.Cout % 32 == 0 && ((int64_t)p.M + 128) * p.Cout * 4 < ((int64_t)1 << 32)),
                 NDET_E_UNSUPPORTED, "%s: the direct epilogue needs splits == 1, no transposition, Cout %% 32 == 0 and an output below 4 GB", fn);
    {
        const int tm = t->rows, tn = t->cols;
        const int64_t mt = (p.M + tm - 1) / tm, nt = (p.Cout + tn - 1) / tn;
        const int64_t taps = p.transposed ? 1 : (int64_t)p.kd * p.kh * p.kw;
        const int64_t w_bytes = taps * p.Cin * p.Cout * 6, a_bytes = (int64_t)p.M * p.Cin * 4 * (p.sd * p.sh * p.sw);
        const int64_t save_w = (mt - 1) * w_bytes, save_a = (nt - 1) * a_bytes;
        p.order = NDET_ORDER_DEFAULT;
        if (NDET_ORDER_DEFAULT < 0) {
            p.order = 0;
            if (!p.transposed && mt > 1 && nt * p.splits > 1 && save_w > save_a && w_bytes > (8 << 20)) p.order = 1;
            if (g_order2 && p.order == 0 && !p.transposed && nt > 1 && mt >= 16 && w_bytes <= (2 << 20) && save_a >= (8 << 20) &&
                (t->flags & NDET_TILE_ORDER2)) p.order = 2;
        }
    }
    const int rc = batch == 1 ? t->launch(p, st, fn) : t->launch_batch(p, batch, st, fn);
    if (rc != NDET_OK) return rc;
    NDET_CHECK_LAUNCH(fn);
    if (keep_partials && p.splits > 1) return NDET_OK;
    return conv_splitk_reduce_launch(p, st, fn);
}
int conv_split_launch(Conv3dParams& p, int tile, bool keep_partials, hipStream_t st, const char* fn) {
    return conv_split_launch_n(p, tile, keep_partials, 1, st, fn);
}

__global__ __launch_bounds__(256) void k_split_weights(const float* __restrict__ w, int taps, int Cout, int Cin, uint16_t* __restrict__ out) {
    const int64_t i = ((int64_t)blockIdx.x * blockDim.x + threadIdx.x) * 2;
    const int64_t n = (int64_t)taps * Cout * Cin;
    if (i >= n) return;
    const int ci = (int)(i % Cin), co = (int)((i / Cin) % Cout), tap = (int)(i / ((int64_t)Cin * Cout));
    const float a = w[i], b = w[i + 1];
    const uint32_t o0 = spl_pack(a, b);
    const float ra = a - spl_lo(o0), rb = b - spl_hi(o0);
    const uint32_t o1 = spl_pack(ra, rb);
    const uint32_t o2 = spl_pack(ra - spl_lo(o1), rb - spl_hi(o1));
    const uint32_t o[3] = {o0, o1, o2};
    const int steps = Cin / CBK;
    uint16_t* dst = out + (((int64_t)tap * steps + ci / CBK) * 3 * Cout + co) * CBK + (ci % CBK);
#pragma unroll
    for (int pl = 0; pl < 3; ++pl) *reinterpret_cast<uint32_t*>(dst + (int64_t)pl * Cout * CBK) = o[pl];
}

extern "C" int ndet_split_weights_bf16x3(const float* w_packed, int taps, int Cout, int Cin, uint16_t* planes, void* stream) {
    const char* fn = "ndet_split_weights_bf16x3";
    NDET_REQUIRE(w_packed && planes, NDET_E_INVALID, "%s: null pointer", fn);
    NDET_REQUIRE(taps > 0 && Cout > 0 && Cin > 0, NDET_E_INVALID, "%s: sizes must be positive", fn);
    NDET_REQUIRE(Cin % CBK == 0, NDET_E_UNSUPPORTED, "%s: Cin=%d must be a multiple of %d", fn, Cin, CBK);
    const int64_t work = (int64_t)taps * Cout * Cin / 2;
    hipLaunchKernelGGL(k_split_weights, dim3((unsigned)((work + 255) / 256)), dim3(256), 0, (hipStream_t)stream, w_packed, taps, Cout, Cin, planes);
    NDET_CHECK_LAUNCH(fn);
    return NDET_OK;
}

__global__ __launch_bounds__(256) void k_split_weights_f16x2(const float* __restrict__ w, int taps, int Cout, int Cin, float scale, uint16_t* __restrict__ out) {
    const int64_t i = ((int64_t)blockIdx.x * blockDim.x + threadIdx.x) * 2;
    const int64_t n = (int64_t)taps * Cout * Cin;
    if (i >= n) return;
    const int ci = (int)(i % Cin), co = (int)((i / Cin) % Cout), tap = (int)(i / ((int64_t)Cin * Cout));
    const float a = w[i] * scale, b = w[i + 1] * scale;
    const uint32_t o0 = spl_pack_f16(a, b);
    const uint32_t o1 = spl_pack_f16(a - spl_f16_lo(o0), b - spl_f16_hi(o0));
    const int steps = Cin / CBK;
    uint16_t* dst = out + (((int64_t)tap * steps + ci / CBK) * 2 * Cout + co) * CBK + (ci % CBK);
    *reinterpret_cast<uint32_t*>(dst) = o0;
    *reinterpret_cast<uint32_t*>(dst + (int64_t)Cout * CBK) = o1;
}

extern "C" int ndet_split_weights_f16x2(const float* w_packed, int taps, int Cout, int Cin, float scale, uint16_t* planes, void* stream) {
    const char* fn = "ndet_split_weights_f16x2";
    NDET_REQUIRE(w_packed && planes, NDET_E_INVALID, "%s: null pointer", fn);
    NDET_REQUIRE(taps > 0 && Cout > 0 && Cin > 0 && scale > 0.0f, NDET_E_INVALID, "%s: sizes and scale must be positive", fn);
    NDET_REQUIRE(Cin % CBK == 0, NDET_E_UNSUPPORTED, "%s: Cin=%d must be a multiple of %d", fn, Cin, CBK);
// ... 178 lines not shown
    p.M = p.OD * p.OH * p.OW;
    return NDET_OK;
}

static int max_order_of(int arith) { return arith == 0 ? 2 : (arith == 1 ? 1 : 0); }

static int conv_split_entry(const NdetConvArgs* a, int batch, void* stream, const char* fn) {
    NDET_REQUIRE(a && a->size == (int32_t)sizeof(NdetConvArgs), NDET_E_INVALID, "%s: the argument block must be set up with size = %d", fn,
                 (int)sizeof(NdetConvArgs));
    NDET_REQUIRE(a->arith >= 0 && a->arith <= 2, NDET_E_INVALID, "%s: arith must be 0 (bf16x3), 1 (fp16 pair) or 2 (bf16)", fn);
    const bool f16 = a->arith == 1, train = a->w_amax != nullptr;
    NDET_REQUIRE(!train || (f16 && !a->transposed && !a->residual_up2), NDET_E_INVALID,
                 "%s: w_amax (the training form) needs arith 1, no transposition and no upsampled residual", fn);
    if (f16) {
        NDET_REQUIRE(a->in_amax && (train || a->w_inv_scale > 0.0f), NDET_E_INVALID,
                     "%s: the fp16-pair arithmetic needs the input's amax slot and the weight planes' inverse scale (or w_amax)", fn);
        NDET_REQUIRE(!a->guard || (a->guard_l1 >= 0.0f && a->guard_tol > 0.0f), NDET_E_INVALID, "%s: the guard needs guard_l1 >= 0 and guard_tol > 0", fn);
    } else {
        NDET_REQUIRE(!a->in_amax, NDET_E_INVALID, "%s: in_amax belongs to the fp16-pair arithmetic only", fn);
    }
    NDET_REQUIRE(!a->keep_partials || (!a->scale && !a->residual && !a->relu && !a->out_amax && !a->transposed), NDET_E_INVALID,
                 "%s: keep_partials leaves the epilogue to ndet_wgrad_to_torch (no affine / residual / ReLU / amax, no transposition)", fn);
    if (a->map_w || a->map_b || a->map_out) {
        NDET_REQUIRE(a->map_w && a->map_b && a->map_out, NDET_E_INVALID, "%s: null projection pointers", fn);
        NDET_REQUIRE((((uintptr_t)a->map_w | (uintptr_t)a->map_b | (uintptr_t)a->map_out) & 15) == 0, NDET_E_UNSUPPORTED,
                     "%s: projection pointers must be 16-byte aligned", fn);
        const ConvTile* t = conv_tile(a->tile);
        NDET_REQUIRE(t && (t->flags & NDET_TILE_OWNS_ROWS), NDET_E_UNSUPPORTED, "%s: tile %d does not own whole rows (3256 / 3257 / 3258 do)", fn, a->tile);
        NDET_REQUIRE(a->Cout == 256, NDET_E_UNSUPPORTED, "%s: Cout=%d, the 256-column tiles own whole rows of 256 channels only", fn, a->Cout);
        NDET_REQUIRE(a->splits <= 1 && !a->residual && !a->relu && !a->transposed, NDET_E_UNSUPPORTED,
                     "%s: the chained projection takes no split-K, residual, ReLU or transposition", fn);
    }
    if (batch != 1) {
        NDET_REQUIRE(batch >= 1, NDET_E_INVALID, "%s: batch=%d must be at least 1", fn, batch);
        NDET_REQUIRE(!a->w_amax && !a->keep_partials && !a->residual_up2 && !a->map_w && !a->map_b && !a->map_out, NDET_E_UNSUPPORTED,
                     "%s: a batch takes no w_amax, keep_partials, upsampled residual or chained projection", fn);
        const ConvTile* t = conv_tile(a->tile);
        NDET_REQUIRE(!t || t->launch_batch, NDET_E_UNSUPPORTED, "%s: tile %d (persistent) takes one volume per launch", fn, a->tile);
    }
    NDET_REQUIRE(a->in && a->w_planes && a->out, NDET_E_INVALID, "%s: null pointer", fn);
    NDET_REQUIRE(a->D > 0 && a->H > 0 && a->W > 0 && a->Cin > 0 && a->Cout > 0, NDET_E_INVALID, "%s: sizes must be positive", fn);
    NDET_REQUIRE((a->scale == nullptr) == (a->shift == nullptr), NDET_E_INVALID, "%s: scale and shift go together", fn);
    NDET_REQUIRE(a->relu >= 0 && a->relu <= 2, NDET_E_INVALID, "%s: bad relu mode", fn);
    NDET_REQUIRE(a->Cin % CBK == 0, NDET_E_UNSUPPORTED, "%s: Cin=%d must be a multiple of %d", fn, a->Cin, CBK);
    NDET_REQUIRE((((uintptr_t)a->in | (uintptr_t)a->w_planes) & 15) == 0, NDET_E_UNSUPPORTED, "%s: in / weights must be 16-byte aligned", fn);
    Conv3dParams p;
    p.in = a->in; p.w = reinterpret_cast<const float*>(a->w_planes); p.out = a->out; p.scale = a->scale; p.shift = a->shift; p.res = a->residual;
    p.partial = (float*)a->workspace;
    p.D = a->D; p.H = a->H; p.W = a->W; p.Cin = a->Cin; p.Cout = a->Cout; p.relu = a->relu;
    p.max_order = max_order_of(a->arith);
    p.amax_in = a->in_amax; p.winv = f16 && !train ? a->w_inv_scale : 1.0f; p.w_amax = a->w_amax; p.amax_out = a->out_amax;
    p.guard = f16 ? a->guard : nullptr; p.guard_l1 = a->guard_l1; p.guard_tol = a->guard_tol;
    p.map_w = a->map_w; p.map_b = a->map_b; p.map_out = a->map_out;
    if (a->transposed) {
        for (int i = 0; i < 3; ++i)
            NDET_REQUIRE(a->kernel[i] == 2 && a->stride[i] == 2 && a->pad[i] == 0, NDET_E_UNSUPPORTED, "%s: transposed conv supports kernel 2 stride 2 pad 0 only", fn);
        p.transposed = 1;
        p.kd = p.kh = p.kw = 2; p.sd = p.sh = p.sw = 2; p.pd = p.ph = p.pw = 0;
        p.OD = 2 * p.D; p.OH = 2 * p.H; p.OW = 2 * p.W;
        NDET_REQUIRE((int64_t)batch * p.OD * p.OH * p.OW < ((int64_t)1 << 31), NDET_E_UNSUPPORTED, "%s: tensor too large", fn);
        p.M = batch * p.D * p.H * p.W;
        p.splits = 1; p.partial = nullptr;
        p.res_up2 = 0; p.RH = p.RW = 0;
        return conv_split_launch_n(p, a->tile, false, batch, (hipStream_t)stream, fn);
    }
    const int rc = conv_geometry(p, a->kernel, a->stride, a->pad, fn);
    if (rc != NDET_OK) return rc;
    NDET_REQUIRE((int64_t)batch * p.M < ((int64_t)1 << 31) && (int64_t)batch * p.D * p.H * p.W * p.Cin < ((int64_t)1 << 40), NDET_E_UNSUPPORTED,
                 "%s: the %d volumes of the batch are too large together", fn, batch);
    p.M *= batch;
    p.splits = a->splits < 1 ? 1 : a->splits;
    p.res_up2 = (a->residual && a->residual_up2) ? 1 : 0;
    p.RH = (p.OH + 1) / 2; p.RW = (p.OW + 1) / 2;
    NDET_REQUIRE(!(p.res_up2 && p.splits > 1), NDET_E_UNSUPPORTED, "%s: upsampled residual cannot be combined with split-K", fn);
    const int iters = p.kd * p.kh * p.kw * (p.Cin / CBK);
    NDET_REQUIRE(p.splits <= iters, NDET_E_INVALID, "%s: splits=%d exceeds the %d K steps", fn, p.splits, iters);
    NDET_REQUIRE(p.splits == 1 || a->workspace != nullptr, NDET_E_INVALID, "%s: split-K needs a workspace", fn);
    return conv_split_launch_n(p, a->tile, a->keep_partials != 0, batch, (hipStream_t)stream, fn);
}
extern "C" int ndet_conv_split(const NdetConvArgs* a, void* stream) { return conv_split_entry(a, 1, stream, "ndet_conv_split"); }
extern "C" int ndet_conv_split_batch(const NdetConvArgs* a, int batch, void* stream) { return conv_split_entry(a, batch, stream, "ndet_conv_split_batch"); }

template <int MID, int SCH>
static int chain_launch(const Conv3dParams& p, const ConvChain& c, hipStream_t st, const char* fn) {
    constexpr int NPL = Spl<SCH>::NPL;
    size_t lds = (size_t)NPL * (128 + MID) * SPL_RS * sizeof(uint16_t);
    const size_t y = (size_t)NPL * (MID == 128 ? 64 : 128) * MID * sizeof(uint16_t);
    if (y > lds) lds = y;
    if (lds > 64 * 1024) NDET_RAISE_LDS((k_conv_split_chain<MID, SCH>), lds);
    hipLaunchKernelGGL((k_conv_split_chain<MID, SCH>), dim3((p.M + 127) / 128), dim3(256), lds, st, p, (const uint16_t*)p.w, c);
    return NDET_OK;
}

extern "C" int ndet_conv_chain(const float* in, const uint16_t* w_planes, int D, int H, int W, int Cin, int Cmid, const int* kernel,
                               const int* stride, const int* pad, const float* scale1, const float* shift1, const uint16_t* w3_planes,
                               int Cout, const float* scale3, const float* shift3, const float* residual, int relu3, float* out,
                               int arith, const float* in_amax, float w1_inv_scale, float w3_inv_scale, float* out_amax, float guard_l1,
                               float guard_l1_3, float guard_tol, unsigned* guard, void* stream) {
    const char* fn = "ndet_conv_chain";
    NDET_REQUIRE(arith >= 0 && arith <= 2, NDET_E_INVALID, "%s: arith must be 0 (bf16x3), 1 (fp16 pair) or 2 (bf16)", fn);
    NDET_REQUIRE((arith == 1) == (in_amax != nullptr), NDET_E_INVALID, "%s: in_amax goes with the fp16-pair arithmetic", fn);
    NDET_REQUIRE(arith != 1 || (w1_inv_scale > 0.0f && w3_inv_scale > 0.0f), NDET_E_INVALID, "%s: the fp16-pair arithmetic needs the weight planes' inverse scales", fn);
    NDET_REQUIRE(arith != 1 || !guard || (guard_l1 >= 0.0f && guard_l1_3 >= 0.0f && guard_tol > 0.0f), NDET_E_INVALID, "%s: the guard needs l1 >= 0 and tol > 0", fn);
    NDET_REQUIRE(in && w_planes && w3_planes && out && kernel && stride && pad, NDET_E_INVALID, "%s: null pointer", fn);
    NDET_REQUIRE(D > 0 && H > 0 && W > 0 && Cin > 0 && Cout > 0, NDET_E_INVALID, "%s: sizes must be positive", fn);
    NDET_REQUIRE((scale1 == nullptr) == (shift1 == nullptr) && (scale3 == nullptr) == (shift3 == nullptr), NDET_E_INVALID, "%s: scale and shift go together", fn);
// ... 89 lines not shown
```

nerf-det_amd/csrc/volume_kernels.hip:

```cpp
#include "ndet_common.hpp"

#include <stdarg.h>

#include <map>
#include <mutex>
#include <utility>

static thread_local char g_err[512] = "";

void ndet_set_error(const char* fmt, ...) {
    va_list ap;
    va_start(ap, fmt);
    vsnprintf(g_err, sizeof(g_err), fmt, ap);
    va_end(ap);
}

hipError_t ndet_lds_limit(const void* kernel, size_t bytes) {
    struct Raised { size_t bytes; hipError_t err; };
    static std::mutex mu;
    static std::map<std::pair<const void*, int>, Raised> seen;
    int dev = 0;
    if (hipGetDevice(&dev) != hipSuccess) dev = 0;
    std::lock_guard<std::mutex> lock(mu);
    const auto it = seen.find({kernel, dev});
    if (it != seen.end() && it->second.bytes >= bytes) return it->second.err;
    const hipError_t e = hipFuncSetAttribute(kernel, hipFuncAttributeMaxDynamicSharedMemorySize, (int)bytes);
    seen[{kernel, dev}] = {bytes, e};
    return e;
}

int g_ndet_deterministic_scatter = 0;
extern "C" int ndet_version(void) { return 110; }
extern "C" const char* ndet_last_error(void) { return g_err; }

#define VOX_PER_TILE 16
#ifndef K2_BATCH
#define K2_BATCH 4
#endif
#ifndef GATHER_BATCH
#define GATHER_BATCH 4
#endif
#ifndef K1_MIN_WAVES
#define K1_MIN_WAVES 6
#endif

__global__ __launch_bounds__(256) void k_get_points(float* __restrict__ pts, int nx, int ny, int nz,
                                                    float vx, float vy, float vz, float ox, float oy, float oz) {
    const int N = nx * ny * nz;
    const int n = blockIdx.x * blockDim.x + threadIdx.x;
    if (n >= N) return;
    const int iz = n % nz;
    const int iy = (n / nz) % ny;
    const int ix = n / (nz * ny);
// ... 236 lines not shown
            const float4 a = pm[0], b = pm[1], c = pm[2];
            P[0] = a.x; P[1] = a.y; P[2] = a.z; P[3] = a.w;
            P[4] = b.x; P[5] = b.y; P[6] = b.z; P[7] = b.w;
            P[8] = c.x; P[9] = c.y; P[10] = c.z; P[11] = c.w;
        }
        int off[VPW];
        unsigned long long mask[VPW];
#pragma unroll
        for (int j = 0; j < VPW; ++j) {
            int xi = 0, yi = 0;
            float z;
            bool ok = (v < n_views) && live[j] && ndet_project_z(P, px[j], py[j], pz[j], w, h, xi, yi, z);
            if (DG) ok = ok && ndet_depth_band(dgate, v, xi, yi, z);
            off[j] = yi * row_pitch + xi * C;
            mask[j] = __ballot(ok);
            cnt[j] += __popcll(mask[j]);
        }
        const float* vbase = feat + (int64_t)r0 * view_pitch;
#pragma unroll
        for (int j = 0; j < VPW; ++j) {
            unsigned long long m = mask[j];
            int b = 0;
            while (m) {
                float4 t[GATHER_BATCH][NCHUNK];
                bool has[GATHER_BATCH];
#pragma unroll
                for (int k = 0; k < GATHER_BATCH; ++k) {
                    has[k] = (m != 0ull);
                    if (has[k]) {
                        b = __builtin_ctzll(m);
                        m &= (m - 1ull);
                    }
                    const int o = __builtin_amdgcn_readlane(off[j], b);
                    const float4* p = reinterpret_cast<const float4*>(vbase + (int64_t)b * view_pitch + o);
#pragma unroll
                    for (int q = 0; q < NCHUNK; ++q) {
                        const int ci = lane + q * 64;
                        t[k][q] = (ci < c4) ? p[ci] : make_float4(0.f, 0.f, 0.f, 0.f);
                    }
                }
#pragma unroll
                for (int k = 0; k < GATHER_BATCH; ++k) {
                    if (has[k]) {
#pragma unroll
                        for (int q = 0; q < NCHUNK; ++q) acc[j][q] = ndet_add4(acc[j][q], t[k][q]);
                    }
                }
            }
        }
    }
}

template <int NCHUNK, bool GATE, int LAYOUT, bool DG>
__global__ __launch_bounds__(256, DG ? K1_MIN_WAVES - 1 : K1_MIN_WAVES) void k_backproject_aggregate(
    const float* __restrict__ feat, int n_views, int C, int h, int w, int64_t view_pitch, int row_pitch,
    const float* __restrict__ points, int N, const float* __restrict__ proj, const float* __restrict__ alpha,
    float* __restrict__ out, int64_t* __restrict__ count, int n_tiles, NdetGateMap dgate) {
    extern __shared__ __attribute__((aligned(16))) float smem[];
    constexpr int VPW = VOX_PER_TILE / 4;
    const int lane = threadIdx.x & 63;
    const int wave = threadIdx.x >> 6;
    const int tile = ndet_xcd_remap(blockIdx.x, n_tiles);
    const int n0 = tile * VOX_PER_TILE;
    const int c4 = C >> 2;
    const int ldp = C + 4;

    float px[VPW], py[VPW], pz[VPW];
    bool live[VPW];
#pragma unroll
    for (int j = 0; j < VPW; ++j) {
        const int n = n0 + j * 4 + wave;
        live[j] = n < N;
        const int nn = live[j] ? n : 0;
        px[j] = points[nn];
        py[j] = points[N + nn];
        pz[j] = points[2 * N + nn];
    }
    float4 acc[VPW][NCHUNK];
    int cnt[VPW];
#pragma unroll
    for (int j = 0; j < VPW; ++j) {
        cnt[j] = 0;
#pragma unroll
        for (int q = 0; q < NCHUNK; ++q) acc[j][q] = make_float4(0.f, 0.f, 0.f, 0.f);
    }

    for (int r0 = 0; r0 < n_views; r0 += 64) {
        const int v = r0 + lane;
        float P[12];
        {
            const float4* pm = reinterpret_cast<const float4*>(proj + (v < n_views ? v : 0) * 12);
            const float4 a = pm[0], b = pm[1], c = pm[2];
            P[0] = a.x; P[1] = a.y; P[2] = a.z; P[3] = a.w;
            P[4] = b.x; P[5] = b.y; P[6] = b.z; P[7] = b.w;
            P[8] = c.x; P[9] = c.y; P[10] = c.z; P[11] = c.w;
        }
        int off[VPW];
        unsigned long long mask[VPW];
#pragma unroll
        for (int j = 0; j < VPW; ++j) {
            int xi = 0, yi = 0;
            float z;
            bool ok = (v < n_views) && live[j] && ndet_project_z(P, px[j], py[j], pz[j], w, h, xi, yi, z);
            if (DG) ok = ok && ndet_depth_band(dgate, v, xi, yi, z);
            off[j] = yi * row_pitch + xi * C;
            mask[j] = __ballot(ok);
            cnt[j] += __popcll(mask[j]);
        }
        const float* vbase = feat + (int64_t)r0 * view_pitch;
#pragma unroll
        for (int j = 0; j < VPW; ++j) {
            unsigned long long m = mask[j];
            int b = 0;
            while (m) {
                float4 t[GATHER_BATCH][NCHUNK];
                bool has[GATHER_BATCH];
#pragma unroll
                for (int k = 0; k < GATHER_BATCH; ++k) {
                    has[k] = (m != 0ull);
                    if (has[k]) {
                        b = __builtin_ctzll(m);
                        m &= (m - 1ull);
                    }
                    const int o = __builtin_amdgcn_readlane(off[j], b);
                    const float4* p = reinterpret_cast<const float4*>(vbase + (int64_t)b * view_pitch + o);
#pragma unroll
                    for (int q = 0; q < NCHUNK; ++q) {
                        const int ci = lane + q * 64;
                        t[k][q] = (ci < c4) ? p[ci] : make_float4(0.f, 0.f, 0.f, 0.f);
                    }
                }
#pragma unroll
                for (int k = 0; k < GATHER_BATCH; ++k) {
                    if (has[k]) {
#pragma unroll
                        for (int q = 0; q < NCHUNK; ++q) acc[j][q] = ndet_add4(acc[j][q], t[k][q]);
                    }
                }
            }
        }
    }

#pragma unroll
    for (int j = 0; j < VPW; ++j) {
        if (!live[j]) continue;
        const int slot = j * 4 + wave;
        const int n = n0 + slot;
        const float denom = (float)cnt[j] + 1e-8f;
        float a = 1.0f;
        if (GATE) a = alpha[n];
#pragma unroll
        for (int q = 0; q < NCHUNK; ++q) {
            float4 mean;
            mean.x = acc[j][q].x / denom;
            mean.y = acc[j][q].y / denom;
            mean.z = acc[j][q].z / denom;
            mean.w = acc[j][q].w / denom;
            if (GATE) {
                mean.x = a * mean.x;
                mean.y = a * mean.y;
                mean.z = a * mean.z;
                mean.w = a * mean.w;
            }
            if (cnt[j] == 0) mean = make_float4(0.f, 0.f, 0.f, 0.f);
            const int ci = lane + q * 64;
            if (ci < c4) {
                if (LAYOUT == NDET_LAYOUT_NC)
                    *reinterpret_cast<float4*>(out + (int64_t)n * C + ci * 4) = mean;
                else
                    *reinterpret_cast<float4*>(smem + slot * ldp + ci * 4) = mean;
            }
        }
        if (lane == 0) count[n] = (int64_t)cnt[j];
    }

    if (LAYOUT == NDET_LAYOUT_CN) {
        __syncthreads();
        for (int idx = threadIdx.x; idx < C * VOX_PER_TILE; idx += 256) {
            const int c = idx >> 4, jv = idx & 15;
            const int n = n0 + jv;
            if (n < N) out[(int64_t)c * N + n] = smem[jv * ldp + c];
        }
    }
}

template <int NCHUNK, bool DG>
static void launch_k1(bool gate, int layout, dim3 grid, size_t lds, hipStream_t st, const float* feat, int n_views, int C,
                      int h, int w, int64_t view_pitch, int row_pitch, const float* points, int N, const float* proj,
                      const float* alpha, float* out, int64_t* count, int n_tiles, const NdetGateMap& dgate) {
#define K1_LAUNCH(G, L)                                                                                                  \
    hipLaunchKernelGGL((k_backproject_aggregate<NCHUNK, G, L, DG>), grid, dim3(256), lds, st, feat, n_views, C, h, w,    \
                       view_pitch, row_pitch, points, N, proj, alpha, out, count, n_tiles, dgate)
    if (gate) {
        if (layout == NDET_LAYOUT_NC) K1_LAUNCH(true, NDET_LAYOUT_NC);
        else K1_LAUNCH(true, NDET_LAYOUT_CN);
    } else {
        if (layout == NDET_LAYOUT_NC) K1_LAUNCH(false, NDET_LAYOUT_NC);
        else K1_LAUNCH(false, NDET_LAYOUT_CN);
    }
#undef K1_LAUNCH
}

static int backproject_aggregate_impl(const char* fn, const float* features_nhwc, int n_views, int C, int h, int w,
                                      int64_t view_pitch, int64_t row_pitch, const float* points, int N,
                                      const float* projection, const float* alpha, float* out, int out_layout,
                                      int64_t* count, const NdetDepthGate* dgate, void* stream) {
    NDET_REQUIRE(features_nhwc && points && projection && out && count, NDET_E_INVALID, "%s: null pointer", fn);
    NDET_REQUIRE(n_views > 0 && C > 0 && h > 0 && w > 0 && N > 0, NDET_E_INVALID, "%s: sizes must be positive", fn);
    NDET_REQUIRE(out_layout == NDET_LAYOUT_CN || out_layout == NDET_LAYOUT_NC, NDET_E_INVALID, "%s: bad layout %d", fn, out_layout);
    NDET_REQUIRE(C % 4 == 0 && C <= 1024, NDET_E_UNSUPPORTED, "%s: C=%d must be a multiple of 4 and <= 1024", fn, C);
    NDET_REQUIRE(row_pitch >= (int64_t)w * C && view_pitch >= (int64_t)h * row_pitch, NDET_E_INVALID, "%s: pitches smaller than the image", fn);
    NDET_REQUIRE(row_pitch % 4 == 0 && view_pitch % 4 == 0 && ((uintptr_t)features_nhwc & 15) == 0, NDET_E_UNSUPPORTED,
                 "%s: feature rows must be 16-byte aligned", fn);
    NDET_REQUIRE((int64_t)h * row_pitch < (int64_t)1 << 31, NDET_E_UNSUPPORTED, "%s: one view exceeds 2^31 floats", fn);
    if (out_layout == NDET_LAYOUT_NC) NDET_REQUIRE(((uintptr_t)out & 15) == 0, NDET_E_UNSUPPORTED, "%s: out must be 16-byte aligned", fn);
    NdetGateMap gm = {};
    if (dgate) {
        const int rc = ndet_gate_prepare(dgate, fn, n_views, h, w, 0, 0, false, &gm, nullptr);
        if (rc != NDET_OK) return rc;
    }
    const int n_tiles = (N + VOX_PER_TILE - 1) / VOX_PER_TILE;
    const size_t lds = out_layout == NDET_LAYOUT_CN ? (size_t)VOX_PER_TILE * (C + 4) * sizeof(float) : 0;
    const dim3 grid(n_tiles);
    hipStream_t st = (hipStream_t)stream;
    const bool gate = alpha != nullptr;
#define K1_CHUNKS(DG)                                                                                                                                \
    if (C <= 256)                                                                                                                                    \
        launch_k1<1, DG>(gate, out_layout, grid, lds, st, features_nhwc, n_views, C, h, w, view_pitch, (int)row_pitch, points, N, projection, alpha, \
                         out, count, n_tiles, gm);                                                                                                   \
    else if (C <= 512)                                                                                                                               \
        launch_k1<2, DG>(gate, out_layout, grid, lds, st, features_nhwc, n_views, C, h, w, view_pitch, (int)row_pitch, points, N, projection, alpha, \
                         out, count, n_tiles, gm);                                                                                                   \
    else                                                                                                                                             \
        launch_k1<4, DG>(gate, out_layout, grid, lds, st, features_nhwc, n_views, C, h, w, view_pitch, (int)row_pitch, points, N, projection, alpha, \
                         out, count, n_tiles, gm)
    if (dgate) {
        K1_CHUNKS(true);
    } else {
        K1_CHUNKS(false);
    }
#undef K1_CHUNKS
    NDET_CHECK_LAUNCH(fn);
    return NDET_OK;
}

extern "C" int ndet_backproject_aggregate(const float* features_nhwc, int n_views, int C, int h, int w,
                                          int64_t view_pitch, int64_t row_pitch, const float* points, int N,
                                          const float* projection, const float* alpha, float* out, int out_layout,
                                          int64_t* count, void* stream) {
    return backproject_aggregate_impl("ndet_backproject_aggregate", features_nhwc, n_views, C, h, w, view_pitch, row_pitch, points, N,
                                      projection, alpha, out, out_layout, count, nullptr, stream);
}

extern "C" int ndet_backproject_aggregate_gated(const float* features_nhwc, int n_views, int C, int h, int w,
                                                int64_t view_pitch, int64_t row_pitch, const float* points, int N,
                                                const float* projection, const float* alpha, float* out, int out_layout,
                                                int64_t* count, const NdetDepthGate* gate, void* stream) {
    NDET_REQUIRE(gate, NDET_E_INVALID, "ndet_backproject_aggregate_gated: null depth gate");
    return backproject_aggregate_impl("ndet_backproject_aggregate_gated", features_nhwc, n_views, C, h, w, view_pitch, row_pitch, points, N,
                                      projection, alpha, out, out_layout, count, gate, stream);
}

template <int NCHUNK, bool DG>
__device__ __forceinline__ void k1_accumulate_body(const float* __restrict__ feat, int n_views, int C, int h, int w, int64_t view_pitch,
                                                   int row_pitch, const float* __restrict__ points, int N, const float* __restrict__ proj,
                                                   float* __restrict__ sum, int pitch, int* __restrict__ count, int n_tiles,
                                                   const NdetGateMap& dgate) {
    constexpr int VPW = K1_VPW;
    const int lane = threadIdx.x & 63;
    const int wave = threadIdx.x >> 6;
    const int tile = ndet_xcd_remap(blockIdx.x, n_tiles);
    const int n0 = tile * VOX_PER_TILE;
    const int c4 = C >> 2;
    float px[VPW], py[VPW], pz[VPW];
    bool live[VPW];
    float4 acc[VPW][NCHUNK];
    int cnt[VPW];
#pragma unroll
    for (int j = 0; j < VPW; ++j) {
        const int n = n0 + j * 4 + wave;
        live[j] = n < N;
        const int nn = live[j] ? n : 0;
        px[j] = points[nn];
        py[j] = points[N + nn];
        pz[j] = points[2 * N + nn];
        cnt[j] = live[j] ? count[nn] : 0;
#pragma unroll
        for (int q = 0; q < NCHUNK; ++q) {
            const int ci = lane + q * 64;
            acc[j][q] = (live[j] && ci < c4) ? *reinterpret_cast<const float4*>(sum + (int64_t)nn * pitch + ci * 4) : make_float4(0.f, 0.f, 0.f, 0.f);
        }
    }
    k1_walk<NCHUNK, DG>(feat, n_views, C, h, w, view_pitch, row_pitch, proj, px, py, pz, live, acc, cnt, dgate, lane);
#pragma unroll
    for (int j = 0; j < VPW; ++j) {
        if (!live[j]) continue;
        const int n = n0 + j * 4 + wave;
#pragma unroll
        for (int q = 0; q < NCHUNK; ++q) {
            const int ci = lane + q * 64;
            if (ci < c4) *reinterpret_cast<float4*>(sum + (int64_t)n * pitch + ci * 4) = acc[j][q];
        }
        if (lane == 0) count[n] = cnt[j];
    }
}

__device__ __forceinline__ void k1_finish_quad(float4 s, int cnt, const float* __restrict__ alpha, int64_t row, int C, int q,
                                               float* __restrict__ out, int64_t* __restrict__ out_count) {
    const float denom = (float)cnt + 1e-8f;
    float4 mean;
    mean.x = s.x / denom;
    mean.y = s.y / denom;
    mean.z = s.z / denom;
// ... 765 lines not shown
```

nerf-det_amd/detector.py:

```python
from __future__ import annotations

import torch
from torch import nn

from . import ops, trace
from .boxes import DepthInstance3DBoxes, bbox3d2result
from .pipeline import IMG_MEAN, IMG_STD
from .radiance_field import VanillaNeRFRadianceField
from .registry import DETECTORS, build_backbone, build_head, build_neck
from .volume import extract_volume, scene_geometry


class BaseDetector(nn.Module):

    def init_weights(self, pretrained=None):
        pass

    def forward(self, img, img_metas, return_loss=True, **kwargs):
        if return_loss:
            return self.forward_train(img, img_metas, **kwargs)
        return self.forward_test(img, img_metas, **kwargs)

    @staticmethod
    def _parse_losses(losses, defer_log=False):
        import torch.distributed as dist
        log = {}
        for k, v in losses.items():
            log[k] = v.mean() if isinstance(v, torch.Tensor) else sum(x.mean() for x in v)
        loss = sum(v for k, v in log.items() if "loss" in k)
        log["loss"] = loss
        out = {}
        for k, v in log.items():
            v = v.detach().clone()
            if dist.is_available() and dist.is_initialized():
                dist.all_reduce(v.div_(dist.get_world_size()))
            out[k] = v if defer_log else v.item()
        return loss, out

    def train_step(self, data, optimizer=None, defer_log=False):
        loss, log_vars = self._parse_losses(self(**data), defer_log)
        return dict(loss=loss, log_vars=log_vars, num_samples=len(data["img_metas"]))


@DETECTORS.register_module()
class nerfdet(BaseDetector):
    def __init__(self, backbone, neck, neck_3d, bbox_head, n_voxels, voxel_size, head_2d=None, train_cfg=None,
                 test_cfg=None, pretrained=None, aabb=None, near_far_range=None, N_samples=40, N_rand=4096,
                 depth_supervise=False, use_nerf_mask=True, nerf_sample_view=3, nerf_mode="volume", squeeze_scale=4,
                 rgb_supervision=True, nerf_density=False, render_testing=False):
        super().__init__()
        assert head_2d is None, "head_2d (SUN RGB-D layout head) is not used by any nerfdet config (nerfdet.py:46)"
        self.backbone = build_backbone(backbone)
        self.neck = build_neck(neck)
        self.neck_3d = build_neck(neck_3d)
        bbox_head = dict(bbox_head)
        bbox_head.update(train_cfg=train_cfg, test_cfg=test_cfg)
        self.bbox_head = build_head(bbox_head)
        self.bbox_head.voxel_size = voxel_size
        self.head_2d = None
# ... 31 lines not shown

    def extract_2d(self, img):
        b = img.shape[0]
        x = img.reshape([-1] + list(img.shape)[2:])
        x = self.neck(self.backbone(x))[0]
        stride = img.shape[-1] / x.shape[-1]
        assert stride == 4
        return x, b, int(stride)

    def extract_feat(self, img, img_metas, mode, depth=None, ray_batch=None):
        if depth is not None:
            assert depth.shape[0] == img.shape[0], "depth and img must hold the same scenes (nerfdet.py:137)"
            depth = depth.reshape([-1] + list(depth.shape)[2:])
        assert ray_batch is not None and self.nerf_density and self.nerf_mode == "image", \
            "effective contract of the reference: use_ray=True, nerf_density=True, nerf_mode='image' (SURVEY.md 0.2)"
        trace.mark("begin")
        draws = begun = None
        if mode == "train":
            from . import rays
            from .rays import begin_selection, collect_draw, submit_draw
            begun = begin_selection(ray_batch)
            if begun is not None and rays.THREADED_DRAW:
                draws = [submit_draw(begun, self.N_rand) for _ in img_metas]
        x, batch, stride = self.extract_2d(img)
        trace.mark("backbone_fpn")
        if begun is not None and draws is None:
            draws = [submit_draw(begun, self.N_rand) for _ in img_metas]
        geoms = None
        if not torch.is_grad_enabled():
            geoms = [scene_geometry(m, self.n_voxels, self.voxel_size, stride, img.device) for m in img_metas]
        n_v = x.shape[0] // batch
        f2d = getattr(x, "_ndet_feature_2d", None)
        denorm = ray_batch["denorm_images"]
        volumes, valids, rgb_preds = [], [], []
        for b, img_meta in enumerate(img_metas):
            feat = x[b * n_v:(b + 1) * n_v]
            dn = denorm.reshape([-1] + list(denorm.shape)[2:])
            hf, wf = img_meta["img_shape"][0] // stride, img_meta["img_shape"][1] // stride
            gated = {} if depth is None else dict(depth=depth[b * n_v:(b + 1) * n_v])
            out = extract_volume(feat, dn, img_meta, self.n_voxels, self.voxel_size, self.mapping, self.nerf_mlp,
                                 stride=stride, channels_last_out=True,
                                 feature_2d=None if (f2d is None or torch.is_grad_enabled()) else f2d[b * n_v:(b + 1) * n_v, :, :hf, :wf],
                                 geometry=None if geoms is None else geoms[b], **gated)
            if mode == "train" or self.render_testing:
                from .rays import render_rays
                rgb_preds.append(render_rays(ray_batch, None, None, out["feature_2d"], dn, self.aabb, self.near_far_range,
                                             self.N_samples, self.N_rand, self.nerf_mlp, img_meta, None, self.nerf_mode,
                                             self.nerf_sample_view, is_train=(mode == "train"),
                                             render_testing=self.render_testing, selection=None if draws is None else collect_draw(draws[b])))
            else:
                rgb_preds.append(None)
            volumes.append(out["volume"])
            valids.append(out["valid"])
        x3 = volumes[0].unsqueeze(0) if len(volumes) == 1 else torch.stack(volumes)
        valids = valids[0].unsqueeze(0) if len(valids) == 1 else torch.stack(valids)
        trace.mark("volumetric_hot_path")
        x3 = self.neck_3d(x3)
        trace.mark("neck3d")
        return x3, valids, None, rgb_preds, []

    @staticmethod
    def _ray_batch(kwargs):
        rb = {}
        if "raydirs" in kwargs:
            rb = dict(ray_o=kwargs["lightpos"], ray_d=kwargs["raydirs"], gt_rgb=kwargs["gt_images"],
                      gt_depth=kwargs["gt_depths"], nerf_sizes=kwargs["nerf_sizes"], denorm_images=kwargs["denorm_images"])
            if kwargs.get("depth_rays") is not None:
                rb["depth_rays"] = kwargs["depth_rays"]
        return rb

    def forward_train(self, img, img_metas, gt_bboxes_3d, gt_labels_3d, **kwargs):
        rb = self._ray_batch(kwargs)
        x, valids, _, rgb_preds, _ = self.extract_feat(img, img_metas, "train", ray_batch=rb or None)
        losses = self.bbox_head.forward_train(x, valids.float(), img_metas, gt_bboxes_3d, gt_labels_3d)
        if rb and self.rgb_supervision:
            losses.update(self.nvs_loss_func(rgb_preds))
        if self.depth_supervise:
            losses.update(self.depth_loss_func(rgb_preds))
        return losses

    def nvs_loss_func(self, rgb_pred):
        loss = 0
        for ret in rgb_pred:
            rgb, gt, m = ret["outputs_coarse"]["rgb"], ret["gt_rgb"], ret["outputs_coarse"]["mask"]
            loss = loss + (torch.sum(m.unsqueeze(-1) * (rgb - gt) ** 2) / (m.sum() + 1e-6) if self.use_nerf_mask
                           else torch.mean((rgb - gt) ** 2))
        return dict(loss_nvs=loss)

    def depth_loss_func(self, rgb_pred):
        loss = 0
        for ret in rgb_pred:
            d, gt, m = ret["outputs_coarse"]["depth"], ret["gt_depth"].squeeze(-1), ret["outputs_coarse"]["mask"]
            loss = loss + (torch.sum(m * torch.abs(d - gt)) / (m.sum() + 1e-6) if self.use_nerf_mask
                           else torch.mean(torch.abs(d - gt)))
        return dict(loss_depth=loss)

    def forward_test(self, img, img_metas, **kwargs):
        rb = self._ray_batch(kwargs)
        return self.simple_test(img, img_metas, ray_batch=rb or None)

    def _repeat_exact(self, img, img_metas, depth, ray_batch, evaluate_nerf):
        from . import conv3d
        conv3d.guard_trips += 1
        prev = conv3d.set_arithmetic("bf16x3")
        try:
            return self.simple_test(img, img_metas, depth, ray_batch, evaluate_nerf, defer=False)
        finally:
# ... 65 lines not shown
```

nerf-det_amd/neck3d.py:

```python
from __future__ import annotations

import torch
from torch import nn
import torch.nn.functional as F

from .conv3d import carry_amax, conv3d_ndhwc, packed, to_ndhwc
from .conv_train import conv_forward
from .registry import NECKS


class BasicBlock3dV2(nn.Module):
    def __init__(self, in_channels, out_channels, stride=1):
        super().__init__()
        self.stride = stride
        self.conv1 = nn.Conv3d(in_channels, out_channels, 3, stride, 1, bias=False)
        self.norm1 = nn.BatchNorm3d(out_channels)
        self.relu = nn.ReLU(inplace=True)
        self.conv2 = nn.Conv3d(out_channels, out_channels, 3, 1, 1, bias=False)
        self.norm2 = nn.BatchNorm3d(out_channels)
        if stride != 1:
            self.downsample = nn.Sequential(nn.Conv3d(in_channels, out_channels, 1, stride, bias=False),
                                            nn.BatchNorm3d(out_channels))

    def forward(self, x):
# ... 40 lines not shown
    return nn.Sequential(nn.Conv3d(cin, cout, 3, 1, 1, bias=False), nn.BatchNorm3d(cout), nn.ReLU(inplace=True))


def _run(seq: nn.Sequential, x):
    mods = list(seq)
    i = 0
    while i < len(mods):
        m = mods[i]
        if isinstance(m, (nn.Conv3d, nn.ConvTranspose3d)):
            x = conv_forward(m, x)
        elif isinstance(m, nn.BatchNorm3d):
            fuse = i + 1 < len(mods) and isinstance(mods[i + 1], nn.ReLU)
            x = _bn(m, x, relu=fuse)
            i += int(fuse)
        else:
            x = m(x)
        i += 1
    return x


@NECKS.register_module()
class FastIndoorImVoxelNeck(nn.Module):
    def __init__(self, in_channels, n_blocks, out_channels):
        super().__init__()
        self.n_scales = len(n_blocks)
        c = in_channels
        for i, nb in enumerate(n_blocks):
            stride = 1 if i == 0 else 2
            blocks = []
            for b in range(nb):
                if b == 0 and stride != 1:
                    blocks.append(BasicBlock3dV2(c, c * 2, stride))
                    c *= 2
                else:
                    blocks.append(BasicBlock3dV2(c, c))
            setattr(self, f"down_layer_{i}", nn.Sequential(*blocks))
            if i > 0:
                setattr(self, f"up_block_{i}", nn.Sequential(
                    nn.ConvTranspose3d(c, c // 2, 2, 2, bias=False), nn.BatchNorm3d(c // 2), nn.ReLU(inplace=True),
                    nn.Conv3d(c // 2, c // 2, 3, 1, 1, bias=False), nn.BatchNorm3d(c // 2), nn.ReLU(inplace=True)))
            setattr(self, f"out_block_{i}", _conv_bn_relu(c, out_channels))

    def init_weights(self):
        pass

    def forward(self, x):
        if x.is_cuda and not self.training and not torch.is_grad_enabled() and x.shape[1] % 32 == 0:
            return self.forward_hip(x)
        return self.forward_library(x)

    def forward_hip(self, x):
        per_level = [[] for _ in range(self.n_scales)]
        for b in range(x.shape[0]):
            t = to_ndhwc(x[b].float())
            downs = []
            for i in range(self.n_scales):
                for blk in getattr(self, f"down_layer_{i}"):
                    t = blk.forward_ndhwc(t)
                downs.append(t)
            for i in range(self.n_scales - 1, -1, -1):
                if i < self.n_scales - 1:
                    up = getattr(self, f"up_block_{i + 1}")
                    t = conv3d_ndhwc(t, packed([up[0]], up[1]), relu=1)
                    t = conv3d_ndhwc(t, packed([up[3]], up[4]), residual=downs[i], relu=2)
                ob = getattr(self, f"out_block_{i}")
                o = conv3d_ndhwc(t, packed([ob[0]], ob[1]), relu=1)
                per_level[i].append(carry_amax(o, o.permute(3, 0, 1, 2)))
        return [carry_amax(lv[0], lv[0].unsqueeze(0)) if len(lv) == 1 else torch.stack(lv) for lv in per_level]

    def forward_batched(self, x):
        t = x.float().permute(0, 2, 3, 4, 1)
        outs = self._levels_ndhwc(carry_amax(x, t if t.is_contiguous() else t.contiguous()))
        return [carry_amax(o, o.permute(0, 4, 1, 2, 3)) for o in outs]

    def _levels_ndhwc(self, t):
        downs, outs = [], [None] * self.n_scales
        for i in range(self.n_scales):
            for blk in getattr(self, f"down_layer_{i}"):
                t = blk.forward_ndhwc(t)
            downs.append(t)
        for i in range(self.n_scales - 1, -1, -1):
            if i < self.n_scales - 1:
                up = getattr(self, f"up_block_{i + 1}")
                t = conv3d_ndhwc(t, packed([up[0]], up[1]), relu=1)
                t = conv3d_ndhwc(t, packed([up[3]], up[4]), residual=downs[i], relu=2)
            ob = getattr(self, f"out_block_{i}")
            outs[i] = conv3d_ndhwc(t, packed([ob[0]], ob[1]), relu=1)
        return outs

    def forward_library(self, x):
        downs = []
        for i in range(self.n_scales):
            x = getattr(self, f"down_layer_{i}")(x)
            downs.append(x)
        outs = []
        for i in range(self.n_scales - 1, -1, -1):
            if i < self.n_scales - 1:
                x = downs[i] + _run(getattr(self, f"up_block_{i + 1}"), x)
            outs.append(_run(getattr(self, f"out_block_{i}"), x))
        return outs[::-1]
```

nerf-det_amd/ops.py:

```python
from __future__ import annotations

import ctypes
import math
from typing import Optional, Sequence, Tuple

import numpy as np
import torch

from . import _lib, trace
from .hostmath import matmul_fma_chain
from ._lib import NDET_LAYOUT_CN, NDET_LAYOUT_NC, NdetDepthGate, NdetSceneAccum, _ptr, _stream, check, float3

Tensor = torch.Tensor


def _need_gpu(*ts: Tensor):
    for t in ts:
        if t is not None and not t.is_cuda:
            raise RuntimeError("nerfdet_amd.ops: tensors must live on the GPU (no CPU fallback in the product path)")


def _f32c(t: Tensor) -> Tensor:
    return t.to(torch.float32).contiguous()

# ... 99 lines not shown
        if r is not None:
            g.H, g.W = r.shape[1], r.shape[2]
            g.depth_r, g.r_view_pitch, g.r_row_pitch = r.data_ptr(), r.stride(0), r.stride(1)
        g.band = self.band
        return g


def depth_gate(depth: Tensor, voxel_size, feat_hw, img_hw=None) -> DepthGate:
    assert voxel_size is not None, "the depth gate needs voxel_size (its band is voxel_size[2], nerfdet.py:408)"
    vs = voxel_size.tolist() if isinstance(voxel_size, Tensor) else list(voxel_size)
    d_f, d_r = depth_resize(depth, feat_hw, img_hw)
    return DepthGate(d_f, d_r, float(vs[-1]))


def _gate_arg(gate: Optional[DepthGate], n_v: int, hw, img_hw=None):
    if gate is None:
        return None
    assert gate.n_views == n_v and tuple(gate.depth_f.shape[1:]) == tuple(hw), \
        f"depth gate for {tuple(gate.depth_f.shape)}, map is {(n_v,) + tuple(hw)}"
    if img_hw is not None:
        assert gate.depth_r is not None and tuple(gate.depth_r.shape[1:]) == tuple(img_hw), "depth gate has no map at the image's size"
    return ctypes.byref(gate.block())


def backproject(features: Tensor, points: Tensor, projection: Tensor, depth=None, voxel_size=None) -> Tuple[Tensor, Tensor]:
    if depth is not None:
        assert isinstance(depth, Tensor) and depth.dim() == 3 and depth.shape[0] == features.shape[0], \
            "depth must be (n_views, H, W) (nerfdet.py:405)"
        assert voxel_size is not None, "depth-gated backproject needs voxel_size (nerfdet.py:408)"
    _need_gpu(features, points, projection, depth)
    if features.dtype != torch.float32:
        features = features.float()
    n_v, c, h, w = features.shape
    gx, gy, gz = points.shape[-3:]
    n = gx * gy * gz
    points = _f32c(points)
    projection = _f32c(projection)
    assert projection.shape == (n_v, 3, 4)
    volume = torch.empty((n_v, c, gx, gy, gz), dtype=torch.float32, device=features.device)
    valid = torch.empty((n_v, 1, gx, gy, gz), dtype=torch.bool, device=features.device)
    sv, sc, sy, sx = features.stride()
    if depth is None:
        check(_lib.load().ndet_backproject(_ptr(features), n_v, c, h, w, sv, sc, sy, sx, _ptr(points), n, _ptr(projection),
                                           _ptr(volume), _ptr(valid), _stream(features)), "backproject")
    else:
        gate = depth_gate(depth, voxel_size, (h, w))
        check(_lib.load().ndet_backproject_gated(_ptr(features), n_v, c, h, w, sv, sc, sy, sx, _ptr(points), n, _ptr(projection),
                                                 _ptr(volume), _ptr(valid), _gate_arg(gate, n_v, (h, w)), _stream(features)), "backproject_gated")
    return volume, valid


def backproject_aggregate(features: Tensor, points: Tensor, projection: Tensor, alpha: Optional[Tensor] = None,
                          channels_last_out: bool = True, out: Optional[Tuple[Tensor, Tensor]] = None,
                          depth_gate: Optional[DepthGate] = None) -> Tuple[Tensor, Tensor]:
    _need_gpu(features, points, projection, alpha)
    f = to_channels_last(features)
    n_v, c, h, w = f.shape
    gx, gy, gz = points.shape[-3:]
    n = gx * gy * gz
    points = _f32c(points)
    projection = _f32c(projection)
    assert projection.shape == (n_v, 3, 4)
    if alpha is not None:
        alpha = _f32c(alpha).reshape(-1)
        assert alpha.numel() == n
    if out is not None:
        vol, count = out
        buf = vol.permute(1, 2, 3, 0) if channels_last_out else vol
        assert buf.is_contiguous() and buf.dtype == torch.float32 and vol.shape == (c, gx, gy, gz)
        assert count.shape == (1, gx, gy, gz) and count.dtype == torch.int64 and count.is_contiguous()
        out, layout = vol, (NDET_LAYOUT_NC if channels_last_out else NDET_LAYOUT_CN)
        from .conv3d import note_raw_write
        note_raw_write(vol)
    else:
        count = torch.empty((1, gx, gy, gz), dtype=torch.int64, device=f.device)
        if channels_last_out:
            buf = torch.empty((gx, gy, gz, c), dtype=torch.float32, device=f.device)
            out, layout = buf.permute(3, 0, 1, 2), NDET_LAYOUT_NC
        else:
            buf = torch.empty((c, gx, gy, gz), dtype=torch.float32, device=f.device)
            out, layout = buf, NDET_LAYOUT_CN
    lib = _lib.load()
    if depth_gate is None:
        launch = lambda: check(lib.ndet_backproject_aggregate(_ptr(f), n_v, c, h, w, f.stride(0), f.stride(2), _ptr(points), n, _ptr(projection),
                                                              _ptr(alpha), _ptr(buf), layout, _ptr(count), _stream(f)), "backproject_aggregate")
    else:
        g = _gate_arg(depth_gate, n_v, (h, w))
        launch = lambda: check(lib.ndet_backproject_aggregate_gated(_ptr(f), n_v, c, h, w, f.stride(0), f.stride(2), _ptr(points), n,
                                                                    _ptr(projection), _ptr(alpha), _ptr(buf), layout, _ptr(count), g, _stream(f)),
                               "backproject_aggregate_gated")
    trace.span("k_backproject_aggregate", launch, bytes=4 * n_v * c * h * w + (4 * c + 8) * n, kind="hbm")
    return out, count


def density_packed_ok(n_views: int, cm: int, mapped: Optional[Tensor] = None, bias: Optional[Tensor] = None) -> bool:
    if cm % 4 or cm > 128 or n_views > 128:
        return False
    if mapped is not None and (mapped.stride(0) % 4 or mapped.stride(2) % 4 or mapped.data_ptr() % 16):
        return False
    return bias is None or bias.data_ptr() % 16 == 0


def density_features(mapped: Tensor, bias: Tensor, denorm_images: Tensor, points: Tensor, projection: Tensor,
                     rgb_projection: Tensor, depth_gate: Optional[DepthGate] = None) -> Tensor:
    _need_gpu(mapped, bias, denorm_images, points, projection, rgb_projection)
    m = to_channels_last(mapped)
    n_v, cm, h, w = m.shape
    rgb = denorm_images if denorm_images.dtype == torch.float32 else denorm_images.float()
    assert rgb.shape[0] == n_v and rgb.shape[1] == 3
    if rgb.stride(3) != 1:
        rgb = rgb.contiguous()
    hh, ww = rgb.shape[2:]
    n = points.shape[-3] * points.shape[-2] * points.shape[-1]
    points, projection, rgb_projection, bias = _f32c(points), _f32c(projection), _f32c(rgb_projection), _f32c(bias)
    out = torch.empty((n, 2 * (3 + cm)), dtype=torch.float32, device=m.device)
    lib = _lib.load()
    packed = density_packed_ok(n_v, cm, m, bias)
    args = (_ptr(m), n_v, cm, h, w, m.stride(0), m.stride(2), _ptr(bias), _ptr(rgb), hh, ww, rgb.stride(0), rgb.stride(1), rgb.stride(2),
            _ptr(points), n, _ptr(projection), _ptr(rgb_projection), _ptr(out))
    if depth_gate is None:
        fn = lib.ndet_density_features_packed if packed else lib.ndet_density_features
        launch = lambda: check(fn(*args, _stream(m)), "density_features")
    else:
        fn = lib.ndet_density_features_packed_gated if packed else lib.ndet_density_features_gated
        g = _gate_arg(depth_gate, n_v, (h, w), (hh, ww))
        launch = lambda: check(fn(*args, g, _stream(m)), "density_features_gated")
    trace.span("k_density_features", launch, bytes=4 * (n_v * 3 * hh * ww + n_v * cm * h * w + 2 * (3 + cm) * n), kind="hbm")
    return out


class SceneState:

    def __init__(self, n_voxels, c: int, cm: int, device):
        self.grid = tuple(int(v) for v in n_voxels)
        n = self.grid[0] * self.grid[1] * self.grid[2]
        assert c % 4 == 0 and cm % 4 == 0, f"streaming needs C and cm in multiples of 4 (got {c}, {cm})"
        self.c, self.cm, self.n_views = int(c), int(cm), 0
        self.k1_sum = torch.zeros((n, c), dtype=torch.float32, device=device)
        self.k1_count = torch.zeros((n,), dtype=torch.int32, device=device)
        self.k2_sum = torch.zeros((n, 3 * (cm + 4)), dtype=torch.float32, device=device)
        self.k2_count = torch.zeros((n, 2), dtype=torch.int32, device=device)

    @property
    def n_voxels(self) -> int:
# ... 561 lines not shown
```

nerf-det_amd/volume.py:

```python
from __future__ import annotations

from typing import Dict, Optional

import torch
import torch.nn.functional as F

from . import ops

Tensor = torch.Tensor


def map_features_2d(features: Tensor, weight: Tensor, bias: Tensor) -> Tensor:
    f = ops.to_channels_last(features)
    rows = f.permute(0, 2, 3, 1)
    if not rows.is_contiguous():
        rows = rows.contiguous()
    from .autograd import LINEAR_ROWS_MIN, LinearRows
    if torch.is_grad_enabled() and rows.is_cuda and rows.numel() // rows.shape[-1] >= LINEAR_ROWS_MIN:
        return LinearRows.apply(rows, weight, bias, False).permute(0, 3, 1, 2)
    return F.linear(rows, weight, bias).permute(0, 3, 1, 2)


def map_features_2d_hip(features: Tensor, lin: torch.nn.Linear) -> Tensor:
    from .conv3d import conv2d_nhwc, packed_linear
    f = ops.to_channels_last(features)
    rows = f.permute(0, 2, 3, 1)
    if not rows.is_contiguous():
        rows = rows.contiguous()
    return conv2d_nhwc(rows, packed_linear(lin), amax=False).permute(0, 3, 1, 2)


def scene_geometry(img_meta: dict, n_voxels, voxel_size, stride: int, device) -> Dict[str, Tensor]:
    return dict(proj=ops.compute_projection(img_meta, stride, device), rgb_proj=ops.compute_projection(img_meta, 1, device),
                points=ops.get_points(n_voxels, voxel_size, img_meta["lidar2img"]["origin"], device))


def density_alpha(features: Tensor, denorm_images: Tensor, img_meta: dict, n_voxels, voxel_size, mapping: torch.nn.Module, nerf_mlp,
                  stride: int = 4, feature_2d: Optional[Tensor] = None, geometry: Optional[Dict[str, Tensor]] = None,
                  depth: Optional[Tensor] = None) -> Dict[str, Tensor]:
    dev = features.device
    h = img_meta["img_shape"][0] // stride
    w = img_meta["img_shape"][1] // stride
    feat = ops.to_channels_last(features)[:, :, :h, :w]
    if geometry is None:
        geometry = scene_geometry(img_meta, n_voxels, voxel_size, stride, dev)
    proj, rgb_proj, pts = geometry["proj"], geometry["rgb_proj"], geometry["points"]
    lin = mapping[0] if isinstance(mapping, torch.nn.Sequential) else mapping
    training = torch.is_grad_enabled() and (feat.requires_grad or lin.weight.requires_grad)
    if feature_2d is None:
        if not training and lin.in_features % 32 == 0:
            feature_2d = map_features_2d_hip(feat, lin)
        else:
            feature_2d = map_features_2d(feat, lin.weight, lin.bias)
    rgb = denorm_images[:, :, :img_meta["img_shape"][0], :img_meta["img_shape"][1]]
    gate = None
    if depth is not None:
        assert depth.dim() == 3 and depth.shape[0] == feat.shape[0], "depth must be the scene's (n_views, H, W) maps (nerfdet.py:136-139)"
        gate = ops.depth_gate(depth.to(dev, non_blocking=True), voxel_size, (h, w), tuple(img_meta["img_shape"][:2]))
    out = dict(feat=feat, feature_2d=feature_2d, points=pts, projection=proj, rgb_projection=rgb_proj, rgb=rgb, lin=lin, depth_gate=gate)
    if training:
        return out
    glob = ops.density_features(feature_2d, lin.bias, rgb, pts, proj, rgb_proj, depth_gate=gate)
    if hasattr(nerf_mlp, "hip_trunk_ok") and nerf_mlp.hip_trunk_ok():
        out.update(global_feat=glob, raw_sigma=None, alpha=nerf_mlp.alpha_from_points(pts, glob))
    else:
        raw_sigma = nerf_mlp.raw_sigma_from_rows(ops.posenc_concat(pts, glob))
        out.update(global_feat=glob, raw_sigma=raw_sigma, alpha=ops.sigma_to_alpha(raw_sigma))
    return out


def extract_volume(features: Tensor, denorm_images: Tensor, img_meta: dict, n_voxels, voxel_size,
                   mapping: torch.nn.Module, nerf_mlp, stride: int = 4, channels_last_out: bool = True,
                   feature_2d: Optional[Tensor] = None, geometry: Optional[Dict[str, Tensor]] = None,
                   depth: Optional[Tensor] = None) -> Dict[str, Tensor]:
    d = density_alpha(features, denorm_images, img_meta, n_voxels, voxel_size, mapping, nerf_mlp, stride, feature_2d, geometry, depth)
    if "alpha" not in d:
        return _extract_volume_train(d["feat"], d["rgb"], d["points"], d["projection"], d["rgb_projection"], d["lin"], nerf_mlp,
                                     d["feature_2d"], channels_last_out, d["depth_gate"])
    volume, count = ops.backproject_aggregate(d["feat"], d["points"], d["projection"], alpha=d["alpha"], channels_last_out=channels_last_out,
                                              depth_gate=d["depth_gate"])
    return dict(volume=volume, valid=count, feature_2d=d["feature_2d"], global_feat=d["global_feat"], raw_sigma=d["raw_sigma"],
                alpha=d["alpha"], points=d["points"], projection=d["projection"], rgb_projection=d["rgb_projection"])


def _extract_volume_train(feat, rgb, pts, proj, rgb_proj, lin, nerf_mlp, feature_2d, channels_last_out, depth_gate=None):
    from .autograd import BackprojectMean, DensityFeatures
    glob = DensityFeatures.apply(feature_2d, lin.bias, rgb, pts, proj, rgb_proj, depth_gate)
    rows = torch.cat([ops.posenc_concat(pts, None), glob], dim=1)
    raw_sigma = nerf_mlp.raw_sigma_from_rows(rows)
    alpha = 1 - torch.exp(-F.relu(raw_sigma))
    mean, count = BackprojectMean.apply(feat, pts, proj, channels_last_out, depth_gate)
    volume = alpha.view(1, *mean.shape[1:]) * mean
    volume = torch.where((count == 0), torch.zeros_like(volume), volume)
    return dict(volume=volume, valid=count, feature_2d=feature_2d, global_feat=glob, raw_sigma=raw_sigma, alpha=alpha.reshape(-1),
                points=pts, projection=proj, rgb_projection=rgb_proj)
```

Before: 146.1 scenes/s.

## Fuse amax into backprojection and add ticket-based in-kernel split-K finish

```diff
diff --git a/include/nerfdet_hip.h b/include/nerfdet_hip.h
--- a/include/nerfdet_hip.h
+++ b/include/nerfdet_hip.h
@@ -74,6 +74,12 @@
                                      const float* points, int N, const float* projection,
                                      const float* alpha, float* out, int out_layout, int64_t* count,
                                      const NdetDepthGate* gate, void* stream);
+
+int ndet_backproject_aggregate_amax(const float* features_nhwc, int n_views, int C, int h, int w,
+                                    int64_t view_pitch, int64_t row_pitch,
+                                    const float* points, int N, const float* projection,
+                                    const float* alpha, float* out, int out_layout, int64_t* count,
+                                    const NdetDepthGate* gate, float* out_amax, void* stream);
 
 int ndet_density_features_gated(const float* mapped_nhwc, int n_views, int cm, int h, int w,
                                 int64_t mview_pitch, int64_t mrow_pitch, const float* bias,
@@ -307,6 +313,8 @@
     unsigned* guard;
     float guard_l1, guard_tol;
     int keep_partials;
+    int n_tickets;
+    int* tickets;
     const float* map_w;
     const float* map_b;
     float* map_out;
diff --git a/nerf-det_amd/_lib.py b/nerf-det_amd/_lib.py
--- a/nerf-det_amd/_lib.py
+++ b/nerf-det_amd/_lib.py
@@ -19,7 +19,7 @@
                 + [(f, c_int * 3) for f in ("kernel", "stride", "pad")] + [("transposed", c_int), ("scale", _P), ("shift", _P), ("residual", _P)]
                 + [(f, c_int) for f in ("residual_up2", "relu", "splits", "tile", "arith")] + [("in_amax", _P), ("w_inv_scale", c_float)]
                 + [(f, _P) for f in ("w_amax", "out_amax", "workspace", "guard")] + [("guard_l1", c_float), ("guard_tol", c_float), ("keep_partials", c_int)]
-                + [(f, _P) for f in ("map_w", "map_b", "map_out")])
+                + [("n_tickets", c_int), ("tickets", _P)] + [(f, _P) for f in ("map_w", "map_b", "map_out")])
 
 
 class NdetDepthGate(ctypes.Structure):
@@ -89,6 +89,7 @@
     "ndet_depth_resize": ([_P, c_int, c_int, c_int, c_int, c_int64, c_int64, _P, c_int, c_int, _P, c_int, c_int, _P], c_int),
     "ndet_backproject_gated": ([_P, c_int, c_int, c_int, c_int, c_int64, c_int64, c_int64, c_int64, _P, c_int, _P, _P, _P, _G, _P], c_int),
     "ndet_backproject_aggregate_gated": ([_P, c_int, c_int, c_int, c_int, c_int64, c_int64, _P, c_int, _P, _P, _P, c_int, _P, _G, _P], c_int),
+    "ndet_backproject_aggregate_amax": ([_P, c_int, c_int, c_int, c_int, c_int64, c_int64, _P, c_int, _P, _P, _P, c_int, _P, _G, _P, _P], c_int),
     "ndet_density_features_gated": ([_P, c_int, c_int, c_int, c_int, c_int64, c_int64, _P, _P, c_int, c_int, c_int64, c_int64,
                                      c_int64, _P, c_int, _P, _P, _P, _G, _P], c_int),
     "ndet_density_features_packed_gated": ([_P, c_int, c_int, c_int, c_int, c_int64, c_int64, _P, _P, c_int, c_int, c_int64, c_int64,
diff --git a/nerf-det_amd/conv3d.py b/nerf-det_amd/conv3d.py
--- a/nerf-det_amd/conv3d.py
+++ b/nerf-det_amd/conv3d.py
@@ -199,6 +199,19 @@
 def guard_tripped(device) -> bool:
     w = guard_word(device)
     return bool(w is not None and int(w.item()) & 1)
+
+
+SPLITK_FINISH = False
+N_TICKETS = 4096
+_TICKETS = {}
+
+
+def splitk_tickets(device) -> torch.Tensor:
+    key = (device, raw_stream(device))
+    t = _TICKETS.get(key)
+    if t is None:
+        t = _TICKETS[key] = torch.zeros(N_TICKETS, dtype=torch.int32, device=device)
+    return t
 
 
 def guard_l1(pk: ConvPack) -> float:
@@ -347,6 +360,8 @@
                           kernel=kernel, stride=stride, pad=pad, transposed=int(transposed), scale=_addr(pk.scale), shift=_addr(pk.shift),
                           residual=_addr(residual), residual_up2=int(residual_up2), relu=relu, splits=splits, tile=tile, arith=ARITH_ID[arith],
                           workspace=_addr(ws))
+    if splits > 1 and (SPLITK_FINISH is True or (SPLITK_FINISH and conv_tiles.TILES[tile].family in SPLITK_FINISH)):
+        a.tickets, a.n_tickets = splitk_tickets(x.device).data_ptr(), N_TICKETS
     keep, mapped = False, None
     if ARITHMETIC != "f16x2":
         a.w_planes = split_planes(pk).data_ptr()
diff --git a/nerf-det_amd/csrc/conv_common.hpp b/nerf-det_amd/csrc/conv_common.hpp
--- a/nerf-det_amd/csrc/conv_common.hpp
+++ b/nerf-det_amd/csrc/conv_common.hpp
@@ -26,6 +26,7 @@
     int max_order;
     int direct = 0;
     int order = 0;
+    int n_tickets = 0;
     const float* amax_in = nullptr;
     float winv = 1.0f;
     const float* w_amax = nullptr;
@@ -37,6 +38,7 @@
     unsigned* guard = nullptr;
     float guard_l1 = 0.0f;
     float guard_tol = 0.0f;
+    int* tickets = nullptr;
 };
 
 
@@ -268,3 +270,76 @@
 }
 
 __device__ __forceinline__ bool conv_writes_final(const Conv3dParams& p) { return p.transposed || p.splits <= 1; }
+
+__device__ __forceinline__ bool conv_splitk_arrive(const Conv3dParams& p, int tile, int* flag, bool first) {
+    asm volatile("s_waitcnt vmcnt(0)" ::: "memory");
+    __syncthreads();
+    if (first) {
+        __builtin_amdgcn_fence(__ATOMIC_RELEASE, "agent");
+        asm volatile("s_waitcnt vmcnt(0)" ::: "memory");
+        const int t = __hip_atomic_fetch_add(p.tickets + tile, 1, __ATOMIC_RELAXED, __HIP_MEMORY_SCOPE_AGENT);
+        const int last = t == p.splits - 1 ? 1 : 0;
+        if (last) {
+            __builtin_amdgcn_fence(__ATOMIC_ACQUIRE, "agent");
+            asm volatile("s_waitcnt vmcnt(0)" ::: "memory");
+        }
+        *flag = last;
+    }
+    __syncthreads();
+    return *flag != 0;
+}
+__device__ __forceinline__ void conv_splitk_release(const Conv3dParams& p, int tile) {
+    __hip_atomic_store(p.tickets + tile, 0, __ATOMIC_RELAXED, __HIP_MEMORY_SCOPE_AGENT);
+}
+
+template <int BN, int NTHR, typename RowMap>
+__device__ __forceinline__ void conv_splitk_finish_rows(const Conv3dParams& p, int rows, int n0, int tid, RowMap m_of, float& mx) {
+    const int64_t MN = (int64_t)p.M * p.Cout;
+    const int S = p.splits;
+    if ((p.Cout & 3) == 0) {
+        constexpr int V = BN / 4;
+        for (int idx = tid; idx < rows * V; idx += NTHR) {
+            const int row = idx / V, c4 = idx % V;
+            const int m = m_of(row), co = n0 + c4 * 4;
+            if (m < 0 || m >= p.M || co >= p.Cout) continue;
+            const int64_t i = (int64_t)m * p.Cout + co;
+            const float* src = p.partial + i;
+            float4 v = *reinterpret_cast<const float4*>(src);
+            for (int s0 = 1; s0 < S; s0 += 4) {
+                float4 t[4];
+#pragma unroll
+                for (int k = 0; k < 4; ++k) t[k] = s0 + k < S ? *reinterpret_cast<const float4*>(src + (int64_t)(s0 + k) * MN) : make_float4(0.f, 0.f, 0.f, 0.f);
+#pragma unroll
+                for (int k = 0; k < 4; ++k)
+                    if (s0 + k < S) { v.x = v.x + t[k].x; v.y = v.y + t[k].y; v.z = v.z + t[k].z; v.w = v.w + t[k].w; }
+            }
+            if (p.scale) {
+                const float4 sc = *reinterpret_cast<const float4*>(p.scale + co), sh = *reinterpret_cast<const float4*>(p.shift + co);
+                v.x = v.x * sc.x + sh.x; v.y = v.y * sc.y + sh.y; v.z = v.z * sc.z + sh.z; v.w = v.w * sc.w + sh.w;
+            }
+            if (p.relu == 2) { v.x = fmaxf(v.x, 0.f); v.y = fmaxf(v.y, 0.f); v.z = fmaxf(v.z, 0.f); v.w = fmaxf(v.w, 0.f); }
+            if (p.res) {
+                const float4 rr = *reinterpret_cast<const float4*>(p.res + i);
+                v.x = v.x + rr.x; v.y = v.y + rr.y; v.z = v.z + rr.z; v.w = v.w + rr.w;
+            }
+            if (p.relu == 1) { v.x = fmaxf(v.x, 0.f); v.y = fmaxf(v.y, 0.f); v.z = fmaxf(v.z, 0.f); v.w = fmaxf(v.w, 0.f); }
+            *reinterpret_cast<float4*>(p.out + i) = v;
+            mx = fmaxf(fmaxf(mx, fmaxf(fabsf(v.x), fabsf(v.y))), fmaxf(fabsf(v.z), fabsf(v.w)));
+        }
+    } else {
+        for (int idx = tid; idx < rows * BN; idx += NTHR) {
+            const int row = idx / BN, c = idx % BN;
+            const int m = m_of(row), co = n0 + c;
+            if (m < 0 || m >= p.M || co >= p.Cout) continue;
+            const int64_t i = (int64_t)m * p.Cout + co;
+            float v = p.partial[i];
+            for (int s = 1; s < S; ++s) v = v + p.partial[(int64_t)s * MN + i];
+            if (p.scale) v = v * p.scale[co] + p.shift[co];
+            if (p.relu == 2) v = fmaxf(v, 0.0f);
+            if (p.res) v = v + p.res[i];
+            if (p.relu == 1) v = fmaxf(v, 0.0f);
+            p.out[i] = v;
+            mx = fmaxf(mx, fabsf(v));
+        }
+    }
+}
diff --git a/nerf-det_amd/csrc/conv_split_kernels.hip b/nerf-det_amd/csrc/conv_split_kernels.hip
--- a/nerf-det_amd/csrc/conv_split_kernels.hip
+++ b/nerf-det_amd/csrc/conv_split_kernels.hip
@@ -186,7 +186,7 @@
 #endif
 template <int BM, int BN, int SCH> constexpr int uni_min_wgs() { return (SCH == 1 && BM == 128 && BN == 128) ? UNI128_F16_WGS : 2; }
 #define SPL_BATCH 4
-template <int BM, int BN, int WGM, int WGN, int SCHB = 0>
+template <int BM, int BN, int WGM, int WGN, int SCHB = 0, bool FIN = false>
 __global__ __launch_bounds__(64 * WGM * WGN, (uni_min_wgs<BM, BN, (SCHB & 3)>())) void k_conv_split(const Conv3dParams p, const uint16_t* __restrict__ wsplit) {
     constexpr int SCH = SCHB & 3;
     constexpr bool BATCH = (SCHB & SPL_BATCH) != 0;
@@ -272,6 +272,14 @@
         __syncthreads();
         conv_store_rows<BN, NTHR>(p, Cs, CLDC, m0 + h * WM, WM, n0, tid, ztap, blk.z, mx, osc);
         __syncthreads();
+    }
+    if constexpr (FIN) {
+        const int tile = blk.y * (int)gridDim.x + blk.x;
+        if (!conv_splitk_arrive(p, tile, reinterpret_cast<int*>(lds16), tid == 0)) return;
+        conv_splitk_finish_rows<BN, NTHR>(p, BM, n0, tid, ConvLinearRows{m0}, mx);
+        if (tid == 0) conv_splitk_release(p, tile);
+        if (p.amax_out) conv_amax_commit(p.amax_out, mx);
+        return;
     }
     if (p.amax_out && conv_writes_final(p)) conv_amax_commit(p.amax_out, mx);
 }
@@ -668,7 +676,7 @@
 #define WS_DEPTH 2
 #define WS_OOB 0x80000000u
 
-template <int SCHB>
+template <int SCHB, bool FIN = false>
 __global__ __launch_bounds__(512, 1) void k_conv_split_ws(const Conv3dParams p, const uint16_t* __restrict__ wsplit) {
     constexpr int SCH = SCHB & 3;
     constexpr bool BATCH = (SCHB & SPL_BATCH) != 0;
@@ -892,6 +900,14 @@
         conv_store_rows<WS_BN, 512>(p, Cs, CLDC, m0 + h * 64, 64, n0, tid, ztap, blk.z, mx, conv_oscale_of(p, amax_in));
         __syncthreads();
     }
+    if constexpr (FIN) {
+        const int tile = blk.y * (int)gridDim.x + blk.x;
+        if (!conv_splitk_arrive(p, tile, reinterpret_cast<int*>(lds16), tid == 0)) return;
+        conv_splitk_finish_rows<WS_BN, 512>(p, WS_BM, n0, tid, ConvLinearRows{m0}, mx);
+        if (tid == 0) conv_splitk_release(p, tile);
+        if (p.amax_out) conv_amax_commit(p.amax_out, mx);
+        return;
+    }
     if (p.amax_out && conv_writes_final(p)) conv_amax_commit(p.amax_out, mx);
 }
 
@@ -916,7 +932,8 @@
     const size_t cs = (size_t)64 * (WS_BN + 4) * sizeof(float);
     if (cs > lds) lds = cs;
     return with_scheme(sch, [&](auto s) -> int {
-        const auto kernel = k_conv_split_ws<decltype(s)::value + (BATCH ? SPL_BATCH : 0)>;
+        constexpr int SCHB = decltype(s)::value + (BATCH ? SPL_BATCH : 0);
+        const auto kernel = p.tickets ? k_conv_split_ws<SCHB, true> : k_conv_split_ws<SCHB, false>;
         NDET_RAISE_LDS(kernel, lds);
         hipLaunchKernelGGL(kernel, grid, dim3(512), lds, st, p, (const uint16_t*)p.w);
         return NDET_OK;
@@ -1264,7 +1281,7 @@
     }
 };
 
-template <int NT16, int WGN, int SCHB, int NPROD = 4>
+template <int NT16, int WGN, int SCHB, int NPROD = 4, bool FIN = false>
 __global__ __launch_bounds__(64 * (2 * WGN + NPROD), 1) void k_conv_split_halo(const Conv3dParams p, const uint16_t* __restrict__ wsplit, const HaloGeom g) {
     constexpr int SCH = SCHB & 3;
     constexpr bool BATCH = (SCHB & SPL_BATCH) != 0;
@@ -1498,6 +1515,16 @@
         else conv_store_rows_mapped<BN, NTHR>(p, Cs, CLDC, 64, n0, tid, 0, blk.z, rmap, mx, osc);
         __syncthreads();
         if (p.map_out) conv_map_rows<BN, NTHR>(p, Cs, CLDC, tid, rmap, osc, Wl);
+    }
+    if constexpr (FIN) {
+        const int tile = blk.y * (int)gridDim.x + blk.x;
+        if (!conv_splitk_arrive(p, tile, reinterpret_cast<int*>(lds16), tid == 0)) return;
+        const HaloRowMap pmap{0, g.ltw, g.lth, d0, h0, w0, p.OD, p.OH, p.OW};
+        if constexpr (BATCH) conv_splitk_finish_rows<BN, NTHR>(p, 128, n0, tid, HaloRowMapBatch{pmap, vol * p.OD * p.OH * p.OW}, mx);
+        else conv_splitk_finish_rows<BN, NTHR>(p, 128, n0, tid, pmap, mx);
+        if (tid == 0) conv_splitk_release(p, tile);
+        if (p.amax_out) conv_amax_commit(p.amax_out, mx);
+        return;
     }
     if (p.amax_out && conv_writes_final(p)) conv_amax_commit(p.amax_out, mx);
 }
@@ -1551,7 +1578,8 @@
                      "%s: the chained projection needs a tile that owns all %d output channels of its rows, no split-K / residual / ReLU", fn, p.Cout);
         lds = lds_cap;
     }
-    const auto kernel = k_conv_split_halo<NT16, WGN, SCH + (BATCH ? SPL_BATCH : 0), NPROD>;
+    const auto kernel = p.tickets ? k_conv_split_halo<NT16, WGN, SCH + (BATCH ? SPL_BATCH : 0), NPROD, true>
+                                  : k_conv_split_halo<NT16, WGN, SCH + (BATCH ? SPL_BATCH : 0), NPROD, false>;
     NDET_RAISE_LDS(kernel, lds_cap);
     hipLaunchKernelGGL(kernel, grid, dim3(64 * (2 * WGN + NPROD)), lds, st, p, (const uint16_t*)p.w, g);
     return NDET_OK;
@@ -1564,7 +1592,8 @@
     size_t lds = (size_t)Spl<SCH>::NPL * (BM + BN) * SPL_RS * sizeof(uint16_t);
     const size_t cs = (size_t)(BM / WGM) * (BN + 4) * sizeof(float);
     if (cs > lds) lds = cs;
-    const auto kernel = k_conv_split<BM, BN, WGM, WGN, SCH + (BATCH ? SPL_BATCH : 0)>;
+    const auto kernel = p.tickets ? k_conv_split<BM, BN, WGM, WGN, SCH + (BATCH ? SPL_BATCH : 0), true>
+                                  : k_conv_split<BM, BN, WGM, WGN, SCH + (BATCH ? SPL_BATCH : 0), false>;
     if (lds > 64 * 1024) NDET_RAISE_LDS(kernel, lds);
     hipLaunchKernelGGL(kernel, grid, dim3(64 * WGM * WGN), lds, st, p, (const uint16_t*)p.w);
     return NDET_OK;
@@ -1671,6 +1700,16 @@
     return NDET_OK;
 }
 
+static int64_t conv_output_tiles(const ConvTile* t, const Conv3dParams& p, int batch) {
+    const int64_t nt = (p.Cout + t->cols - 1) / t->cols;
+    if (t->id == 3128 || (t->flags & NDET_TILE_OWNS_ROWS)) {
+        HaloGeom g;
+        if (!halo_geometry(p, t->cols == 128 ? 400 : 224, g)) return INT64_MAX;
+        return (int64_t)batch * g.npd * g.nph * g.npw * nt;
+    }
+    return (int64_t)((p.M + t->rows - 1) / t->rows) * nt;
+}
+
 static int conv_split_launch_n(Conv3dParams& p, int tile, bool keep_partials, int batch, hipStream_t st, const char* fn) {
     p.nt = (p.splits <= 1 || p.transposed) && (int64_t)p.M * p.Cout * 4 * (p.transposed ? 8 : 1) >= conv_nt_bytes() ? 1 : 0;
     const int64_t big_tiles = (int64_t)((p.M + 127) / 128) * ((p.Cout + 127) / 128);
@@ -1695,10 +1734,11 @@
                 (t->flags & NDET_TILE_ORDER2)) p.order = 2;
         }
     }
+    if (p.tickets && (p.splits <= 1 || p.transposed || keep_partials || !t->launch_batch || conv_output_tiles(t, p, batch) > p.n_tickets)) p.tickets = nullptr;
     const int rc = batch == 1 ? t->launch(p, st, fn) : t->launch_batch(p, batch, st, fn);
     if (rc != NDET_OK) return rc;
     NDET_CHECK_LAUNCH(fn);
-    if (keep_partials && p.splits > 1) return NDET_OK;
+    if ((keep_partials && p.splits > 1) || p.tickets) return NDET_OK;
     return conv_splitk_reduce_launch(p, st, fn);
 }
 int conv_split_launch(Conv3dParams& p, int tile, bool keep_partials, hipStream_t st, const char* fn) {
@@ -1983,6 +2023,8 @@
     p.amax_in = a->in_amax; p.winv = f16 && !train ? a->w_inv_scale : 1.0f; p.w_amax = a->w_amax; p.amax_out = a->out_amax;
     p.guard = f16 ? a->guard : nullptr; p.guard_l1 = a->guard_l1; p.guard_tol = a->guard_tol;
     p.map_w = a->map_w; p.map_b = a->map_b; p.map_out = a->map_out;
+    NDET_REQUIRE(!a->tickets || (a->n_tickets > 0 && ((uintptr_t)a->tickets & 3) == 0), NDET_E_INVALID, "%s: tickets needs n_tickets > 0 aligned counters", fn);
+    p.tickets = a->tickets; p.n_tickets = a->tickets ? a->n_tickets : 0;
     if (a->transposed) {
         for (int i = 0; i < 3; ++i)
             NDET_REQUIRE(a->kernel[i] == 2 && a->stride[i] == 2 && a->pad[i] == 0, NDET_E_UNSUPPORTED, "%s: transposed conv supports kernel 2 stride 2 pad 0 only", fn);
diff --git a/nerf-det_amd/csrc/volume_kernels.hip b/nerf-det_amd/csrc/volume_kernels.hip
--- a/nerf-det_amd/csrc/volume_kernels.hip
+++ b/nerf-det_amd/csrc/volume_kernels.hip
@@ -1,4 +1,5 @@
 #include "ndet_common.hpp"
+#include "conv_common.hpp"
 
 #include <stdarg.h>
 
@@ -341,10 +342,10 @@
 }
 
 template <int NCHUNK, bool GATE, int LAYOUT, bool DG>
-__global__ __launch_bounds__(256, DG ? K1_MIN_WAVES - 1 : K1_MIN_WAVES) void k_backproject_aggregate(
+__global__ __launch_bounds__(256, DG ? K1_MIN_WAVES - 1 : (NCHUNK == 1 ? K1_MIN_WAVES + 1 : K1_MIN_WAVES)) void k_backproject_aggregate(
     const float* __restrict__ feat, int n_views, int C, int h, int w, int64_t view_pitch, int row_pitch,
     const float* __restrict__ points, int N, const float* __restrict__ proj, const float* __restrict__ alpha,
-    float* __restrict__ out, int64_t* __restrict__ count, int n_tiles, NdetGateMap dgate) {
+    float* __restrict__ out, int64_t* __restrict__ count, int n_tiles, NdetGateMap dgate, float* __restrict__ amax_out) {
     extern __shared__ __attribute__((aligned(16))) float smem[];
     constexpr int VPW = VOX_PER_TILE / 4;
     const int lane = threadIdx.x & 63;
@@ -430,6 +431,7 @@
         }
     }
 
+    float vmax = 0.0f;
 #pragma unroll
     for (int j = 0; j < VPW; ++j) {
         if (!live[j]) continue;
@@ -454,6 +456,7 @@
             if (cnt[j] == 0) mean = make_float4(0.f, 0.f, 0.f, 0.f);
             const int ci = lane + q * 64;
             if (ci < c4) {
+                vmax = fmaxf(fmaxf(vmax, fmaxf(fabsf(mean.x), fabsf(mean.y))), fmaxf(fabsf(mean.z), fabsf(mean.w)));
                 if (LAYOUT == NDET_LAYOUT_NC)
                     *reinterpret_cast<float4*>(out + (int64_t)n * C + ci * 4) = mean;
                 else
@@ -471,15 +474,16 @@
             if (n < N) out[(int64_t)c * N + n] = smem[jv * ldp + c];
         }
     }
+    if (amax_out) conv_amax_commit(amax_out, vmax);
 }
 
 template <int NCHUNK, bool DG>
 static void launch_k1(bool gate, int layout, dim3 grid, size_t lds, hipStream_t st, const float* feat, int n_views, int C,
                       int h, int w, int64_t view_pitch, int row_pitch, const float* points, int N, const float* proj,
-                      const float* alpha, float* out, int64_t* count, int n_tiles, const NdetGateMap& dgate) {
+                      const float* alpha, float* out, int64_t* count, int n_tiles, const NdetGateMap& dgate, float* amax_out) {
 #define K1_LAUNCH(G, L)                                                                                                  \
     hipLaunchKernelGGL((k_backproject_aggregate<NCHUNK, G, L, DG>), grid, dim3(256), lds, st, feat, n_views, C, h, w,    \
-                       view_pitch, row_pitch, points, N, proj, alpha, out, count, n_tiles, dgate)
+                       view_pitch, row_pitch, points, N, proj, alpha, out, count, n_tiles, dgate, amax_out)
     if (gate) {
         if (layout == NDET_LAYOUT_NC) K1_LAUNCH(true, NDET_LAYOUT_NC);
         else K1_LAUNCH(true, NDET_LAYOUT_CN);
@@ -493,7 +497,7 @@
 static int backproject_aggregate_impl(const char* fn, const float* features_nhwc, int n_views, int C, int h, int w,
                                       int64_t view_pitch, int64_t row_pitch, const float* points, int N,
                                       const float* projection, const float* alpha, float* out, int out_layout,
-                                      int64_t* count, const NdetDepthGate* dgate, void* stream) {
+                                      int64_t* count, const NdetDepthGate* dgate, float* out_amax, void* stream) {
     NDET_REQUIRE(features_nhwc && points && projection && out && count, NDET_E_INVALID, "%s: null pointer", fn);
     NDET_REQUIRE(n_views > 0 && C > 0 && h > 0 && w > 0 && N > 0, NDET_E_INVALID, "%s: sizes must be positive", fn);
     NDET_REQUIRE(out_layout == NDET_LAYOUT_CN || out_layout == NDET_LAYOUT_NC, NDET_E_INVALID, "%s: bad layout %d", fn, out_layout);
@@ -516,13 +520,13 @@
 #define K1_CHUNKS(DG)                                                                                                                                \
     if (C <= 256)                                                                                                                                    \
         launch_k1<1, DG>(gate, out_layout, grid, lds, st, features_nhwc, n_views, C, h, w, view_pitch, (int)row_pitch, points, N, projection, alpha, \
-                         out, count, n_tiles, gm);                                                                                                   \
+                         out, count, n_tiles, gm, out_amax);                                                                                                   \
     else if (C <= 512)                                                                                                                               \
         launch_k1<2, DG>(gate, out_layout, grid, lds, st, features_nhwc, n_views, C, h, w, view_pitch, (int)row_pitch, points, N, projection, alpha, \
-                         out, count, n_tiles, gm);                                                                                                   \
+                         out, count, n_tiles, gm, out_amax);                                                                                                   \
     else                                                                                                                                             \
         launch_k1<4, DG>(gate, out_layout, grid, lds, st, features_nhwc, n_views, C, h, w, view_pitch, (int)row_pitch, points, N, projection, alpha, \
-                         out, count, n_tiles, gm)
+                         out, count, n_tiles, gm, out_amax)
     if (dgate) {
         K1_CHUNKS(true);
     } else {
@@ -538,7 +542,16 @@
                                           const float* projection, const float* alpha, float* out, int out_layout,
                                           int64_t* count, void* stream) {
     return backproject_aggregate_impl("ndet_backproject_aggregate", features_nhwc, n_views, C, h, w, view_pitch, row_pitch, points, N,
-                                      projection, alpha, out, out_layout, count, nullptr, stream);
+                                      projection, alpha, out, out_layout, count, nullptr, nullptr, stream);
+}
+
+extern "C" int ndet_backproject_aggregate_amax(const float* features_nhwc, int n_views, int C, int h, int w,
+                                               int64_t view_pitch, int64_t row_pitch, const float* points, int N,
+                                               const float* projection, const float* alpha, float* out, int out_layout,
+                                               int64_t* count, const NdetDepthGate* gate, float* out_amax, void* stream) {
+    NDET_REQUIRE(out_amax, NDET_E_INVALID, "ndet_backproject_aggregate_amax: null amax slot");
+    return backproject_aggregate_impl("ndet_backproject_aggregate_amax", features_nhwc, n_views, C, h, w, view_pitch, row_pitch, points, N,
+                                      projection, alpha, out, out_layout, count, gate, out_amax, stream);
 }
 
 extern "C" int ndet_backproject_aggregate_gated(const float* features_nhwc, int n_views, int C, int h, int w,
@@ -547,7 +560,7 @@
                                                 int64_t* count, const NdetDepthGate* gate, void* stream) {
     NDET_REQUIRE(gate, NDET_E_INVALID, "ndet_backproject_aggregate_gated: null depth gate");
     return backproject_aggregate_impl("ndet_backproject_aggregate_gated", features_nhwc, n_views, C, h, w, view_pitch, row_pitch, points, N,
-                                      projection, alpha, out, out_layout, count, gate, stream);
+                                      projection, alpha, out, out_layout, count, gate, nullptr, stream);
 }
 
 template <int NCHUNK, bool DG>
diff --git a/nerf-det_amd/detector.py b/nerf-det_amd/detector.py
--- a/nerf-det_amd/detector.py
+++ b/nerf-det_amd/detector.py
@@ -5,6 +5,7 @@
 
 from . import ops, trace
 from .boxes import DepthInstance3DBoxes, bbox3d2result
+from .conv3d import carry_amax
 from .pipeline import IMG_MEAN, IMG_STD
 from .radiance_field import VanillaNeRFRadianceField
 from .registry import DETECTORS, build_backbone, build_head, build_neck
@@ -142,7 +143,7 @@
                 rgb_preds.append(None)
             volumes.append(out["volume"])
             valids.append(out["valid"])
-        x3 = volumes[0].unsqueeze(0) if len(volumes) == 1 else torch.stack(volumes)
+        x3 = carry_amax(volumes[0], volumes[0].unsqueeze(0)) if len(volumes) == 1 else torch.stack(volumes)
         valids = valids[0].unsqueeze(0) if len(valids) == 1 else torch.stack(valids)
         trace.mark("volumetric_hot_path")
         x3 = self.neck_3d(x3)
diff --git a/nerf-det_amd/neck3d.py b/nerf-det_amd/neck3d.py
--- a/nerf-det_amd/neck3d.py
+++ b/nerf-det_amd/neck3d.py
@@ -116,7 +116,7 @@
     def forward_hip(self, x):
         per_level = [[] for _ in range(self.n_scales)]
         for b in range(x.shape[0]):
-            t = to_ndhwc(x[b].float())
+            t = to_ndhwc(carry_amax(x, x[b]) if (x.shape[0] == 1 and x.dtype == torch.float32) else x[b].float())
             downs = []
             for i in range(self.n_scales):
                 for blk in getattr(self, f"down_layer_{i}"):
diff --git a/nerf-det_amd/ops.py b/nerf-det_amd/ops.py
--- a/nerf-det_amd/ops.py
+++ b/nerf-det_amd/ops.py
@@ -175,7 +175,7 @@
 
 def backproject_aggregate(features: Tensor, points: Tensor, projection: Tensor, alpha: Optional[Tensor] = None,
                           channels_last_out: bool = True, out: Optional[Tuple[Tensor, Tensor]] = None,
-                          depth_gate: Optional[DepthGate] = None) -> Tuple[Tensor, Tensor]:
+                          depth_gate: Optional[DepthGate] = None, amax: bool = False) -> Tuple[Tensor, Tensor]:
     _need_gpu(features, points, projection, alpha)
     f = to_channels_last(features)
     n_v, c, h, w = f.shape
@@ -204,7 +204,15 @@
             buf = torch.empty((c, gx, gy, gz), dtype=torch.float32, device=f.device)
             out, layout = buf, NDET_LAYOUT_CN
     lib = _lib.load()
-    if depth_gate is None:
+    slot = None
+    if amax:
+        from . import conv3d
+        slot = conv3d.AMAX.take(f.device)
+        g = None if depth_gate is None else _gate_arg(depth_gate, n_v, (h, w))
+        launch = lambda: check(lib.ndet_backproject_aggregate_amax(_ptr(f), n_v, c, h, w, f.stride(0), f.stride(2), _ptr(points), n, _ptr(projection),
+                                                                   _ptr(alpha), _ptr(buf), layout, _ptr(count), g, _ptr(slot), _stream(f)),
+                               "backproject_aggregate_amax")
+    elif depth_gate is None:
         launch = lambda: check(lib.ndet_backproject_aggregate(_ptr(f), n_v, c, h, w, f.stride(0), f.stride(2), _ptr(points), n, _ptr(projection),
                                                               _ptr(alpha), _ptr(buf), layout, _ptr(count), _stream(f)), "backproject_aggregate")
     else:
@@ -213,6 +221,8 @@
                                                                     _ptr(projection), _ptr(alpha), _ptr(buf), layout, _ptr(count), g, _stream(f)),
                                "backproject_aggregate_gated")
     trace.span("k_backproject_aggregate", launch, bytes=4 * n_v * c * h * w + (4 * c + 8) * n, kind="hbm")
+    if slot is not None:
+        conv3d._tag_amax(out, slot)
     return out, count
 
 
diff --git a/nerf-det_amd/volume.py b/nerf-det_amd/volume.py
--- a/nerf-det_amd/volume.py
+++ b/nerf-det_amd/volume.py
@@ -8,6 +8,8 @@
 from . import ops
 
 Tensor = torch.Tensor
+
+K1_AMAX = True
 
 
 def map_features_2d(features: Tensor, weight: Tensor, bias: Tensor) -> Tensor:
@@ -77,8 +79,9 @@
     if "alpha" not in d:
         return _extract_volume_train(d["feat"], d["rgb"], d["points"], d["projection"], d["rgb_projection"], d["lin"], nerf_mlp,
                                      d["feature_2d"], channels_last_out, d["depth_gate"])
+    from . import conv3d
     volume, count = ops.backproject_aggregate(d["feat"], d["points"], d["projection"], alpha=d["alpha"], channels_last_out=channels_last_out,
-                                              depth_gate=d["depth_gate"])
+                                              depth_gate=d["depth_gate"], amax=K1_AMAX and conv3d.ARITHMETIC == "f16x2" and not conv3d.NO_AMAX_COMMIT)
     return dict(volume=volume, valid=count, feature_2d=d["feature_2d"], global_feat=d["global_feat"], raw_sigma=d["raw_sigma"],
                 alpha=d["alpha"], points=d["points"], projection=d["projection"], rgb_projection=d["rgb_projection"])
 
```

Result: no change. 145.9 scenes/s (median of 2 runs) (-0.2%).
